# EffortlessMetrics/BitNet-rs

Measured on AMD Instinct MI355X. Metric: decode tokens/sec + I2_S matmul HBM GB/s (% roofline), bitnet-b1.58-2B-4T, higher is better.
Workload: dtype i8 MFMA on producer-quantised activations (QAct: 15-bit fixed point per element, one power-of-two scale per 16), exact integer partial sums, f32 accumulate / f32 elsewhere (f16 embedding table); 1 GPU; bitnet-b1.58-2B-4T I2_S BitNet32-F16 (ternary, one f16 scale per 32 weights), 1xMI355X, batch=1 decode, 128-token prompt; layers=30, prompt_len=128, parallelism=single GPU, launch=hipGraph replay per token, kv_cache=f32 (as the reference, T:1171-1202)

## Files before the change

### bitnet-rs_amd/__init__.py

```python
from __future__ import annotations

import collections
import ctypes as C
import importlib.util
import os
import sys

import numpy as np

HERE = os.path.dirname(os.path.abspath(__file__))
ROOT = os.path.dirname(HERE)
LIB_PATH = os.path.join(HERE, "libbitnet_hip.so")
HEADER_PATH = os.path.join(ROOT, "include", "bitnet_hip.h")

OK = 0
ERR_INVALID_ARGUMENT, ERR_GPU, ERR_UNSUPPORTED, ERR_EXECUTION = -1, -2, -3, -4
KERNEL_AUTO, KERNEL_EXACT, KERNEL_VALU, KERNEL_MFMA, KERNEL_MFMA_TILED = 0, 1, 2, 3, 4
QTYPE_I2S, QTYPE_TL1, QTYPE_TL2 = 0, 1, 2

_u8p = C.POINTER(C.c_uint8)
_i8p = C.POINTER(C.c_int8)
_f32p = C.POINTER(C.c_float)
_sz = C.c_size_t
_vp = C.c_void_p
# ... 18 lines not shown
    spec.loader.exec_module(mod)
    return mod


def build(force: bool = False, verbose: bool = False) -> str:
    return _load_build_module().build(force=force, verbose=verbose)


class DeviceInfo(C.Structure):
    _fields_ = [
        ("device_id", C.c_int32),
        ("name", C.c_char * 128),
        ("gcn_arch", C.c_char * 64),
        ("total_memory", C.c_uint64),
        ("compute_unit_count", C.c_int32),
        ("max_wavefront_size", C.c_int32),
        ("max_shared_memory_per_workgroup", C.c_uint64),
        ("supports_fp16", C.c_int32),
        ("supports_bf16", C.c_int32),
    ]


def _np(a, dtype):
    if isinstance(a, (bytes, bytearray, memoryview)):
        a = np.frombuffer(a, dtype=np.uint8)
    return np.ascontiguousarray(a, dtype=dtype)


def _ptr(t):
    return _vp(t if isinstance(t, int) else t.data_ptr())


def _optr(t):
    return None if t is None else _ptr(t)


class HipLib:

    def __init__(self, path: str = LIB_PATH):
        if not os.path.exists(path):
            raise FileNotFoundError(
                f"{path} not found: build it with __graft_entry__.build() -- there is no fallback path"
            )
        self.path = path
        self.c = C.CDLL(path)
        L = self.c
        L.bitnet_hip_init.argtypes = [C.c_int]
        L.bitnet_hip_cleanup.restype = None
        L.bitnet_hip_get_last_error.restype = C.c_char_p
        L.bitnet_hip_get_device_info.argtypes = [C.c_int, C.POINTER(DeviceInfo)]
        L.bitnet_hip_set_kernel.argtypes = [C.c_int]
        L.bitnet_hip_gemv_qk256.argtypes = [_u8p, _sz, _f32p, _sz, _f32p, _sz, _sz, _sz, _sz]
        L.bitnet_hip_i2s_matmul_f32.argtypes = [_f32p, _sz, _u8p, _sz, _f32p, _sz, _f32p, _sz, _sz, _sz, _sz, _sz]
        L.bitnet_hip_qk256_gemv.argtypes = [_u8p, _sz, _f32p, _sz, _f32p, _sz, _f32p, _sz, _sz, _sz, _sz]
        L.bitnet_hip_matmul_i2s.argtypes = [_i8p, _sz, _u8p, _sz, _f32p, _sz, _sz, _sz, _sz]
        L.bitnet_hip_quantize.argtypes = [_f32p, _sz, _u8p, _sz, _f32p, _sz, C.c_int]
        L.bitnet_hip_dequant_i2s.argtypes = [_u8p, _sz, _sz, _sz, C.c_int, C.c_float, C.c_int, _f32p, _sz]
        L.bitnet_hip_attention.argtypes = [_f32p, _sz, _f32p, _sz, _f32p, _sz, _f32p, _sz, _sz, _sz, _sz, C.c_int, C.c_float]
        L.bitnet_hip_qk256_gemv_batch.argtypes = [C.c_void_p, _sz]
        L.bitnet_hip_weights_upload_qk256.argtypes = [_u8p, _sz, _sz, _sz, _sz, C.POINTER(C.c_uint64)]
        L.bitnet_hip_weights_upload_i2s.argtypes = [_u8p, _sz, _f32p, _sz, _sz, _sz, _sz, C.POINTER(C.c_uint64)]
        L.bitnet_hip_weights_upload_coded.argtypes = [_u8p, _sz, _f32p, _sz, _sz, _sz, _sz, _i8p, C.POINTER(C.c_uint64)]
        L.bitnet_hip_weights_upload_inline_f16.argtypes = [_u8p, _sz, _sz, _sz, _i8p, C.c_int, C.POINTER(C.c_uint64)]
        L.bitnet_hip_weights_free.argtypes = [C.c_uint64]
        L.bitnet_hip_weights_info.argtypes = [C.c_uint64, C.POINTER(_sz), C.POINTER(_sz), C.POINTER(_sz)]
        L.bitnet_hip_gemv_dev.argtypes = [C.c_uint64, _vp, _vp, _vp]
        L.bitnet_hip_matmul_dev.argtypes = [C.c_uint64, _vp, _vp, _sz, _vp]
        L.bitnet_hip_matmul_kernel_dev.argtypes = [C.c_uint64, _vp, _vp, _sz, C.c_int, _vp]
        L.bitnet_hip_add_dev.argtypes = [_vp, _vp, _vp, _sz, _vp]
        L.bitnet_hip_silu_mul_dev.argtypes = [_vp, _vp, _vp, _sz, _sz, _vp]
        L.bitnet_hip_weights_device_bytes.argtypes = [C.c_uint64]
        L.bitnet_hip_weights_device_bytes.restype = _sz
        L.bitnet_hip_weights_trim.argtypes = [C.c_uint64]
        L.bitnet_hip_qact_bytes.argtypes = [_sz]
        L.bitnet_hip_qact_bytes.restype = _sz
        L.bitnet_hip_qact_stats_bytes.argtypes = [_sz]
        L.bitnet_hip_qact_stats_bytes.restype = _sz
        L.bitnet_hip_quantize_act_dev.argtypes = [_vp, _vp, _sz, _vp, _vp, _vp]
        L.bitnet_hip_embed_q_dev.argtypes = [_vp, _vp, _vp, _sz, _sz, _vp, _vp, _vp, _vp, _vp]
        L.bitnet_hip_gemv_q_supported.argtypes = [C.c_uint64]
        L.bitnet_hip_gemv_q_dev.argtypes = [C.c_uint64, _vp, _vp, _vp, C.c_float, _vp, C.c_int, _vp, _vp, _vp, _vp, _vp]
        L.bitnet_hip_attention_decode_q_dev.argtypes = [_vp, _vp, _vp, _vp, _vp, _sz, _sz, _sz, _sz, _vp, _vp, C.c_int, _vp, _vp, _vp]
        L.bitnet_hip_gemv_attn_merge_q_dev.argtypes = [C.c_uint64, _vp, _sz, _sz, _sz, _vp, _vp, _vp, _vp, _vp, _vp, _vp]
        L.bitnet_hip_matmul_workspace_bytes.argtypes = [_sz, _sz, C.c_int]
        L.bitnet_hip_matmul_workspace_bytes.restype = _sz
        L.bitnet_hip_matmul_fused_dev.argtypes = [C.c_uint64, _vp, _vp, _sz, _vp, C.c_float, _vp, C.c_int, C.c_int, _vp, _sz, _vp]
        L.bitnet_hip_matmul_last_tile.argtypes = [C.POINTER(C.c_int)] * 4
        L.bitnet_hip_matmul_last_wave_rows.argtypes = []
        L.bitnet_hip_weights_bind_ln.argtypes = [C.c_uint64, _vp, _vp]
        L.bitnet_hip_weights_concat.argtypes = [C.POINTER(C.c_uint64), _sz, C.c_int, C.POINTER(C.c_uint64)]
        L.bitnet_hip_gemv_fused_dev.argtypes = [C.c_uint64, _vp, _vp, _sz, _vp, C.c_float, _vp, C.c_int, _vp]
        L.bitnet_hip_rmsnorm.argtypes = [_f32p, _sz, _f32p, _sz, _f32p, _sz, _sz, _sz, C.c_float]
        L.bitnet_hip_norm_rows_dev.argtypes = [_vp, _vp, _vp, _sz, _sz, C.c_float, C.c_int, _vp]
        L.bitnet_hip_embed_f16_dev.argtypes = [_vp, _vp, _vp, _sz, _sz, _sz, _vp, _vp]
        L.bitnet_hip_advance_pos_dev.argtypes = [_vp, _vp]
        L.bitnet_hip_attention_decode_dev.argtypes = [_vp, _vp, _vp, _vp, _vp, _sz, _sz, _sz, _sz, _vp, _vp, _vp, _vp]
        L.bitnet_hip_attention_decode_wide_dev.argtypes = [_vp, _vp, _vp, _vp, _vp, _sz, _sz, _sz, _sz, _vp, _vp, _vp, _vp]
        L.bitnet_hip_attention_decode_partial_dev.argtypes = [_vp, _vp, _vp, _vp, _vp, _sz, _sz, _sz, _sz, _vp, _vp, _vp]
        L.bitnet_hip_gemv_attn_merge_dev.argtypes = [C.c_uint64, _vp, _sz, _sz, _sz, _vp, _vp, _vp, _vp]
        L.bitnet_hip_attention_prefill_workspace_bytes.argtypes = [_sz, _sz, _sz]
        L.bitnet_hip_attention_prefill_workspace_bytes.restype = _sz
        L.bitnet_hip_attention_prefill_dev.argtypes = [_vp, _vp, _vp, _vp, _vp, _sz, _sz, _sz, _sz, _sz, _vp, _sz, _vp, _vp]
        L.bitnet_hip_attention_extend_workspace_bytes.argtypes = [_sz, _sz, _sz, _sz]
        L.bitnet_hip_attention_extend_workspace_bytes.restype = _sz
        L.bitnet_hip_attention_extend_dev.argtypes = [_vp, _vp, _vp, _vp, _vp, _sz, _sz, _sz, _sz, _sz, _sz, _vp, _sz, _vp, C.c_int, _vp]
        L.bitnet_hip_attention_prefill_sharded_workspace_bytes.argtypes = [_sz, _sz, _sz, _sz]
        L.bitnet_hip_attention_prefill_sharded_workspace_bytes.restype = _sz
        L.bitnet_hip_attention_prefill_sharded_dev.argtypes = [_vp, _sz, _vp, _sz, _vp, _sz, _sz, _vp, _vp, _vp, _vp, _sz, _sz, _sz, _sz, _vp, _sz, _vp, _vp]
        L.bitnet_hip_attention_scratch_bytes.argtypes = [_sz, _sz]
        L.bitnet_hip_attention_scratch_bytes.restype = _sz
        L.bitnet_hip_logits_f16_dev.argtypes = [_vp, _vp, _vp, C.c_float, _sz, _sz, _vp, _vp, _sz, _vp, _vp, _vp, _vp, _vp]
        L.bitnet_hip_argmax_dev.argtypes = [_vp, _sz, _vp, _sz, _vp, _vp]
        L.bitnet_hip_hbm_read_ceiling.argtypes = [_sz, C.c_int, C.POINTER(C.c_double), C.POINTER(C.c_double), _vp]
        L.bitnet_hip_sampler_create.argtypes = [_sz, C.POINTER(SamplingConfig), C.POINTER(_vp)]
        L.bitnet_hip_sampler_destroy.argtypes = [_vp]
        L.bitnet_hip_sampler_destroy.restype = None
        L.bitnet_hip_sampler_configure.argtypes = [_vp, C.POINTER(SamplingConfig)]
        L.bitnet_hip_sampler_reset.argtypes = [_vp]
        L.bitnet_hip_sampler_draws.argtypes = [_vp, C.POINTER(C.c_uint64)]
        L.bitnet_hip_sample_dev.argtypes = [_vp, _vp, _sz, _vp, _vp, _vp, _vp, _vp]
        L.bitnet_hip_sample_host.argtypes = [_vp, _f32p, _sz, C.POINTER(C.c_uint32), _sz, C.POINTER(C.c_uint32)]
        L.bitnet_hip_score_workspace_bytes.argtypes = [_sz, _sz, _sz]
        L.bitnet_hip_score_workspace_bytes.restype = _sz
        L.bitnet_hip_score_f16_dev.argtypes = [_vp, _vp, _vp, C.c_float, _sz, _sz, _sz, _vp, _vp, _vp, _vp, _sz, _vp, _sz, _vp]

    def last_error(self) -> str:
        e = self.c.bitnet_hip_get_last_error()
        return e.decode() if e else ""

    def _check(self, rc: int) -> None:
        if rc != 0:
            raise BitNetHipError(rc, self.last_error() or f"bitnet_hip rc={rc}")

    def init(self, device: int = -1) -> None:
        self._check(self.c.bitnet_hip_init(device))

    def cleanup(self) -> None:
        self.c.bitnet_hip_cleanup()

    def is_available(self) -> bool:
        return bool(self.c.bitnet_hip_is_available())

    def device_count(self) -> int:
        return int(self.c.bitnet_hip_device_count())

    def device_info(self, device: int = 0) -> DeviceInfo:
        info = DeviceInfo()
        self._check(self.c.bitnet_hip_get_device_info(device, C.byref(info)))
        return info

    def set_kernel(self, kernel: int) -> None:
        self._check(self.c.bitnet_hip_set_kernel(kernel))

    def get_kernel(self) -> int:
        return int(self.c.bitnet_hip_get_kernel())

    def gemv_qk256(self, qs, x, rows, cols, row_stride_bytes, y_len=None) -> np.ndarray:
        q, xa = _np(qs, np.uint8), _np(x, np.float32)
        y = np.zeros(rows if y_len is None else y_len, np.float32)
        self._check(
            self.c.bitnet_hip_gemv_qk256(
                q.ctypes.data_as(_u8p), q.size, xa.ctypes.data_as(_f32p), xa.size, y.ctypes.data_as(_f32p), y.size,
                rows, cols, row_stride_bytes,
            )
        )
        return y
# ... 185 lines not shown
                                                           _vp(stream)))

    def attention_prefill_sharded_workspace_bytes(self, n_heads: int, n_kv: int, n_q: int, n_ctx: int) -> int:
        return int(self.c.bitnet_hip_attention_prefill_sharded_workspace_bytes(n_heads, n_kv, n_q, n_ctx))

    def attention_prefill_sharded_dev(self, q, ld_q, q_block_pos, n_q, kv, ld_kv, n_ctx, rope_sin, rope_cos, kcache, vcache, n_heads, n_kv,
                                      head_dim, max_pos, workspace, workspace_bytes, out, stream: int = 0) -> None:
        self._check(self.c.bitnet_hip_attention_prefill_sharded_dev(_ptr(q), ld_q, _ptr(q_block_pos), n_q, _ptr(kv), ld_kv, n_ctx, _ptr(rope_sin),
                                                                    _ptr(rope_cos), _ptr(kcache), _ptr(vcache), n_heads, n_kv, head_dim, max_pos,
                                                                    _ptr(workspace), workspace_bytes, _ptr(out), _vp(stream)))

    def attention_prefill_gathered_dev(self, q, ld_q, q_block_pos, n_q, kv_gathered, n_ctx, world, kv_is_f16, rope_sin, rope_cos, kcache, vcache,
                                       cache_f16, n_heads, n_kv, head_dim, max_pos, workspace, workspace_bytes, out, stream: int = 0) -> None:
        self.c.bitnet_hip_attention_prefill_gathered_dev.argtypes = [_vp, _sz, _vp, _sz, _vp, _sz, _sz, C.c_int, _vp, _vp, _vp, _vp, C.c_int, _sz, _sz,
                                                                     _sz, _sz, _vp, _sz, _vp, _vp]
        self._check(self.c.bitnet_hip_attention_prefill_gathered_dev(_ptr(q), ld_q, _ptr(q_block_pos), n_q, _ptr(kv_gathered), n_ctx, world,
                                                                     int(kv_is_f16), _ptr(rope_sin), _ptr(rope_cos), _ptr(kcache), _ptr(vcache),
                                                                     int(cache_f16), n_heads, n_kv, head_dim, max_pos, _ptr(workspace), workspace_bytes,
                                                                     _ptr(out), _vp(stream)))

    def weights_bind_ln(self, h: int, ln_gamma, stream: int = 0) -> None:
        self._check(self.c.bitnet_hip_weights_bind_ln(h, _ptr(ln_gamma), _vp(stream)))

    def weights_free(self, h: int) -> None:
        self._check(self.c.bitnet_hip_weights_free(h))

    def weights_info(self, h: int):
        r, c, b = _sz(0), _sz(0), _sz(0)
        self._check(self.c.bitnet_hip_weights_info(h, C.byref(r), C.byref(c), C.byref(b)))
        return r.value, c.value, b.value

    def gemv_dev(self, h: int, x, y, stream: int = 0) -> None:
        self._check(self.c.bitnet_hip_gemv_dev(h, _ptr(x), _ptr(y), _vp(stream)))

    def matmul_dev(self, h: int, x, y, m: int, stream: int = 0) -> None:
        self._check(self.c.bitnet_hip_matmul_dev(h, _ptr(x), _ptr(y), m, _vp(stream)))

    def matmul_kernel_dev(self, h: int, x, y, m: int, kernel: int, stream: int = 0) -> None:
        self._check(self.c.bitnet_hip_matmul_kernel_dev(h, _ptr(x), _ptr(y), m, kernel, _vp(stream)))

    def add_dev(self, a, b, out, n: int, stream: int = 0) -> None:
        self._check(self.c.bitnet_hip_add_dev(_ptr(a), _ptr(b), _ptr(out), n, _vp(stream)))

    def silu_mul_dev(self, gate, up, out, n: int, tile: int = 0, stream: int = 0) -> None:
        self._check(self.c.bitnet_hip_silu_mul_dev(_ptr(gate), _ptr(up), _ptr(out), n, tile, _vp(stream)))

    def weights_device_bytes(self, h: int) -> int:
        return int(self.c.bitnet_hip_weights_device_bytes(h))

    def weights_fp4_image(self, h: int, enable: bool = True, stream: int = 0) -> None:
        self.c.bitnet_hip_weights_fp4_image.argtypes = [C.c_uint64, C.c_int, C.c_void_p]
        self._check(self.c.bitnet_hip_weights_fp4_image(h, 1 if enable else 0, stream))

    def weights_trim(self, h: int) -> None:
        self._check(self.c.bitnet_hip_weights_trim(h))

    def qact_bytes(self, cols: int) -> int:
        return int(self.c.bitnet_hip_qact_bytes(cols))

    def qact_stats_bytes(self, cols: int) -> int:
        return int(self.c.bitnet_hip_qact_stats_bytes(cols))

    def quantize_act_dev(self, x, gamma, cols: int, qact_out, stats_out=None, stream: int = 0) -> None:
        self._check(self.c.bitnet_hip_quantize_act_dev(_ptr(x), _optr(gamma), cols, _ptr(qact_out), _optr(stats_out), _vp(stream)))

    def embed_q_dev(self, table, tokens, x_out, hidden: int, vocab: int, gamma, qact_out, stats_out=None, offset=None, stream: int = 0) -> None:
        self._check(self.c.bitnet_hip_embed_q_dev(_ptr(table), _ptr(tokens), _optr(offset), hidden, vocab, _ptr(x_out), _optr(gamma), _ptr(qact_out),
                                                  _optr(stats_out), _vp(stream)))

    def gemv_q_supported(self, h: int) -> bool:
        return bool(self.c.bitnet_hip_gemv_q_supported(h))

    def gemv_q_dev(self, h: int, qact_in, y=None, stats_in=None, ln_gamma=None, ln_eps: float = 0.0, residual=None, flags: int = 0, qact_out=None,
                   gamma_out=None, stats_out=None, stream: int = 0) -> None:
        self._check(self.c.bitnet_hip_gemv_q_dev(h, _ptr(qact_in), _optr(stats_in), _optr(ln_gamma), ln_eps, _optr(residual), flags, _optr(y),
                                                 _optr(qact_out), _optr(gamma_out), _optr(stats_out), _vp(stream)))

    def attention_decode_q_dev(self, qkv, rope_sin, rope_cos, kcache, vcache, n_heads, n_kv, head_dim, max_pos, pos, scratch, out, qact_out,
                               wide: bool = False, kv_f16: bool = False, stream: int = 0, partial: bool = False) -> None:
        flags = (1 if wide else 0) | (2 if kv_f16 else 0) | (4 if partial else 0)
        self._check(self.c.bitnet_hip_attention_decode_q_dev(_ptr(qkv), _ptr(rope_sin), _ptr(rope_cos), _ptr(kcache), _ptr(vcache), n_heads, n_kv,
                                                             head_dim, max_pos, _ptr(pos), _ptr(scratch), flags, _optr(out), _optr(qact_out), _vp(stream)))

    def gemv_attn_merge_q_dev(self, h: int, scratch, n_heads, n_kv, max_pos, pos, y, qact_out, residual=None, gamma_out=None, stats_out=None,
                              stream: int = 0) -> None:
        self._check(self.c.bitnet_hip_gemv_attn_merge_q_dev(h, _ptr(scratch), n_heads, n_kv, max_pos, _ptr(pos), _ptr(y), _optr(residual),
                                                            _ptr(qact_out), _optr(gamma_out), _optr(stats_out), _vp(stream)))

    def weights_concat(self, parts, interleave16: bool = False) -> int:
        arr = (C.c_uint64 * len(parts))(*parts)
        h = C.c_uint64(0)
        self._check(self.c.bitnet_hip_weights_concat(arr, len(parts), int(interleave16), C.byref(h)))
        return h.value

    def gemv_fused_dev(self, h: int, x, y, m: int = 1, ln_gamma=None, ln_eps: float = 0.0, residual=None, flags: int = 0, stream: int = 0) -> None:
        self._check(
            self.c.bitnet_hip_gemv_fused_dev(h, _ptr(x), _ptr(y), m, _ptr(ln_gamma) if ln_gamma is not None else None, ln_eps,
                                             _ptr(residual) if residual is not None else None, flags, _vp(stream))
        )

    def rmsnorm(self, x, gamma, num_rows: int, hidden: int, eps: float = 1e-6) -> np.ndarray:
        xa, ga = _np(x, np.float32), _np(gamma, np.float32)
        out = np.zeros(num_rows * hidden, np.float32)
        self._check(self.c.bitnet_hip_rmsnorm(xa.ctypes.data_as(_f32p), xa.size, ga.ctypes.data_as(_f32p), ga.size, out.ctypes.data_as(_f32p), out.size, num_rows, hidden, eps))
        return out

    def norm_rows_dev(self, x, gamma, out, rows: int, hidden: int, eps: float, rms: bool, stream: int = 0) -> None:
        self._check(self.c.bitnet_hip_norm_rows_dev(_ptr(x), _ptr(gamma), _ptr(out), rows, hidden, eps, int(rms), _vp(stream)))

    def embed_f16_dev(self, table, tokens, out, n: int, hidden: int, vocab: int, offset=None, stream: int = 0) -> None:
        self._check(self.c.bitnet_hip_embed_f16_dev(_ptr(table), _ptr(tokens), _ptr(offset) if offset is not None else None, n, hidden, vocab, _ptr(out), _vp(stream)))

    def attention_decode_dev(self, qkv, rope_sin, rope_cos, kcache, vcache, n_heads, n_kv, head_dim, max_pos, pos, scratch, out, stream: int = 0) -> None:
        self._check(self.c.bitnet_hip_attention_decode_dev(_ptr(qkv), _ptr(rope_sin), _ptr(rope_cos), _ptr(kcache), _ptr(vcache), n_heads, n_kv, head_dim, max_pos, _ptr(pos), _ptr(scratch), _ptr(out), _vp(stream)))

    def attention_decode_wide_dev(self, qkv, rope_sin, rope_cos, kcache, vcache, n_heads, n_kv, head_dim, max_pos, pos, scratch, out, stream: int = 0) -> None:
        self._check(self.c.bitnet_hip_attention_decode_wide_dev(_ptr(qkv), _ptr(rope_sin), _ptr(rope_cos), _ptr(kcache), _ptr(vcache), n_heads, n_kv, head_dim, max_pos, _ptr(pos), _ptr(scratch), _ptr(out), _vp(stream)))

    def attention_decode_partial_dev(self, qkv, rope_sin, rope_cos, kcache, vcache, n_heads, n_kv, head_dim, max_pos, pos, scratch, stream: int = 0) -> None:
        self._check(self.c.bitnet_hip_attention_decode_partial_dev(_ptr(qkv), _ptr(rope_sin), _ptr(rope_cos), _ptr(kcache), _ptr(vcache), n_heads, n_kv, head_dim, max_pos, _ptr(pos), _ptr(scratch), _vp(stream)))

    def gemv_attn_merge_dev(self, h: int, scratch, n_heads: int, n_kv: int, max_pos: int, pos, y, residual=None, stream: int = 0) -> None:
        self._check(self.c.bitnet_hip_gemv_attn_merge_dev(h, _ptr(scratch), n_heads, n_kv, max_pos, _ptr(pos), _ptr(y), _ptr(residual) if residual is not None else None, _vp(stream)))

    def logits_f16_dev(self, table, x, gamma, eps, hidden, vocab, logits, scratch, n_wg, token=None, pos=None, history=None, n_forced=None, stream: int = 0) -> None:
        opt = lambda t: _ptr(t) if t is not None else None
        self._check(self.c.bitnet_hip_logits_f16_dev(_ptr(table), _ptr(x), opt(gamma), eps, hidden, vocab, _ptr(logits), _ptr(scratch), n_wg, opt(token), opt(pos), opt(history), opt(n_forced), _vp(stream)))

    def score_workspace_bytes(self, n_rows: int, hidden: int, vocab: int) -> int:
        return int(self.c.bitnet_hip_score_workspace_bytes(n_rows, hidden, vocab))

    def score_f16_dev(self, table, x, gamma, eps: float, hidden: int, vocab: int, n_rows: int, targets, nll, argmax=None, logits=None,
                      logits_rows: int = 0, workspace=None, workspace_bytes: int = 0, stream: int = 0) -> None:
        self._check(self.c.bitnet_hip_score_f16_dev(_optr(table), _optr(x), _optr(gamma), eps, hidden, vocab, n_rows, _optr(targets), _optr(nll),
                                                    _optr(argmax), _optr(logits), logits_rows, _optr(workspace), workspace_bytes, _vp(stream)))

    def argmax_dev(self, v, n: int, scratch, n_wg: int, token, stream: int = 0) -> None:
        self._check(self.c.bitnet_hip_argmax_dev(_ptr(v), n, _ptr(scratch), n_wg, _ptr(token), _vp(stream)))

    def sampler(self, vocab: int, temperature: float = 1.0, top_k: int = 0, top_p: float = 1.0, repetition_penalty: float = 1.0,
                seed: int | None = None) -> "Sampler":
        return Sampler(self, vocab, SamplingConfig.make(temperature, top_k, top_p, repetition_penalty, seed))

    def hbm_read_ceiling(self, nbytes: int = 2 << 30, iters: int = 10, stream: int = 0):
        best, mean = C.c_double(0.0), C.c_double(0.0)
        self._check(self.c.bitnet_hip_hbm_read_ceiling(nbytes, iters, C.byref(best), C.byref(mean), _vp(stream)))
        return best.value, mean.value


class SamplingConfig(C.Structure):
    _fields_ = [("temperature", C.c_float), ("top_k", C.c_int32), ("top_p", C.c_float), ("repetition_penalty", C.c_float), ("seed", C.c_uint64)]

    @classmethod
    def make(cls, temperature: float, top_k: int, top_p: float, repetition_penalty: float, seed: int | None = None) -> "SamplingConfig":
        if seed is None:
            seed = int.from_bytes(os.urandom(8), "little")
        return cls(float(temperature), int(top_k), float(top_p), float(repetition_penalty), int(seed) & 0xFFFFFFFFFFFFFFFF)


class Sampler:

    def __init__(self, lib: HipLib, vocab: int, cfg: SamplingConfig):
        self.lib, self.vocab = lib, int(vocab)
        h = _vp()
        lib._check(lib.c.bitnet_hip_sampler_create(vocab, C.byref(cfg), C.byref(h)))
        self.h = h
# ... 112 lines not shown
            self._buf = np.frombuffer(data, np.uint8).copy()
            self.h = L.bitnet_host_gguf_from_memory(self._buf.ctypes.data_as(_u8p), self._buf.size)
        if (path is not None or data is not None) and not self.h:
            raise BitNetHipError(ERR_INVALID_ARGUMENT, self.error() or "GGUF parse failed")

    def error(self) -> str:
        e = self.c.bitnet_host_gguf_error()
        return e.decode(errors="replace") if e else ""

    def close(self) -> None:
        if self.h:
            self.c.bitnet_host_gguf_close(self.h)
            self.h = None

    @property
    def data_start(self) -> int:
        return int(self.c.bitnet_host_gguf_data_start(self.h))

    def tensors(self) -> list:
        out = []
        for i in range(self.c.bitnet_host_gguf_tensor_count(self.h)):
            name = C.create_string_buffer(512)
            shape = (C.c_uint64 * 8)()
            nd, ty, off, size = C.c_uint32(0), C.c_uint32(0), C.c_uint64(0), C.c_uint64(0)
            rc = self.c.bitnet_host_gguf_tensor_info(self.h, i, name, 512, shape, C.byref(nd), C.byref(ty), C.byref(off), C.byref(size))
            if rc != 0:
                raise BitNetHipError(ERR_INVALID_ARGUMENT, self.error())
            out.append({"name": name.value.decode(), "shape": tuple(int(shape[j]) for j in range(nd.value)), "type": ty.value,
                        "offset": off.value, "size": size.value})
        return out

    def config(self) -> dict:
        cfg, f = (C.c_uint64 * 6)(), (C.c_float * 2)()
        if self.c.bitnet_host_gguf_config(self.h, cfg, f) != 0:
            raise BitNetHipError(ERR_INVALID_ARGUMENT, self.error())
        keys = ("vocab", "hidden", "n_layers", "n_heads", "n_kv_heads", "ffn")
        d = {k: int(cfg[i]) for i, k in enumerate(keys)}
        d["rope_theta"] = None if f[0] != f[0] else float(f[0])
        d["eps"] = None if f[1] != f[1] else float(f[1])
        return d

    def detect_i2s_flavor(self, available: int, nelems: int, has_scale_sibling: bool, strict: bool = False) -> str:
        rc = self.c.bitnet_host_gguf_detect_i2s_flavor(available, nelems, int(has_scale_sibling), int(strict))
        if rc < 0:
            raise BitNetHipError(ERR_INVALID_ARGUMENT, self.error())
        return FLAVORS[rc]

    def check_projection(self, idx: int, rows: int, cols: int) -> None:
        if self.c.bitnet_host_gguf_check_projection(self.h, idx, rows, cols) != 0:
            raise BitNetHipError(ERR_INVALID_ARGUMENT, self.error())

    def loader_is_qk256(self, shape, available: int) -> bool:
        sh = (C.c_uint64 * len(shape))(*shape)
        return bool(self.c.bitnet_host_gguf_loader_is_qk256(sh, len(shape), available))


ScoreResult = collections.namedtuple("ScoreResult", "nll argmax logits ms")


class HostDecoder:

    def __init__(self, cfg, path: str = HOST_LIB_PATH):
        if not os.path.exists(path):
            raise FileNotFoundError(f"{path} not found: build it with __graft_entry__.build() -- there is no fallback path")
        load()
        self.c = C.CDLL(path)
        L = self.c
        L.bitnet_host_create.restype = C.c_void_p
        L.bitnet_host_create.argtypes = [C.POINTER(HostConfig)]
        L.bitnet_host_destroy.argtypes = [C.c_void_p]
        L.bitnet_host_error.restype = C.c_char_p
        L.bitnet_host_error.argtypes = [C.c_void_p]
        L.bitnet_host_set_layer_qk256.argtypes = [C.c_void_p, C.c_int, _f32p, _f32p] + [_u8p] * 7
        L.bitnet_host_set_layer_i2s.argtypes = [C.c_void_p, C.c_int, _f32p, _f32p, C.POINTER(_u8p), C.POINTER(_f32p), _sz]
        L.bitnet_host_set_globals.argtypes = [C.c_void_p, C.POINTER(C.c_uint16), _f32p]
        L.bitnet_host_reset.argtypes = [C.c_void_p]
        L.bitnet_host_feed.argtypes = [C.c_void_p, C.POINTER(C.c_int32), C.c_int]
        L.bitnet_host_run.argtypes = [C.c_void_p, C.c_int, C.c_int, C.c_int, C.POINTER(C.c_float)]
        L.bitnet_host_run_reference.argtypes = [C.c_void_p, C.c_int, C.c_int]
        L.bitnet_host_prepare_graphs.argtypes = [C.c_void_p, C.c_int]
        L.bitnet_host_set_act_mode.argtypes = [C.c_void_p, C.c_int]
        L.bitnet_host_act_mode.argtypes = [C.c_void_p]
        L.bitnet_host_position.argtypes = [C.c_void_p]
        L.bitnet_host_last_prefill_path.argtypes = [C.c_void_p]
        L.bitnet_host_saturation_fallbacks.argtypes = [C.c_void_p]
        L.bitnet_host_history.argtypes = [C.c_void_p, C.POINTER(C.c_int32), C.c_int]
        L.bitnet_host_last_logits.argtypes = [C.c_void_p, _f32p]
        L.bitnet_host_last_hidden.argtypes = [C.c_void_p, _f32p]
        L.bitnet_host_probe_gateup.argtypes = [C.c_void_p, C.c_int, C.POINTER(C.c_float), C.POINTER(C.c_double)]
        L.bitnet_host_probe_kernel.argtypes = [C.c_void_p, C.c_int, C.c_int, C.POINTER(C.c_float), C.POINTER(C.c_double)]
        L.bitnet_host_weight_bytes.argtypes = [C.c_void_p]
        L.bitnet_host_weight_bytes.restype = C.c_uint64
        L.bitnet_host_set_sampling.argtypes = [C.c_void_p, C.POINTER(SamplingConfig)]
        L.bitnet_host_sampling_draws.argtypes = [C.c_void_p, C.POINTER(C.c_uint64)]
        L.bitnet_host_score.argtypes = [C.c_void_p, C.c_int, C.c_int, _f32p, C.POINTER(C.c_int32), _f32p, C.c_int, C.POINTER(C.c_float)]
        L.bitnet_host_extend.argtypes = [C.c_void_p, C.c_int, C.c_int, C.c_int, C.POINTER(C.c_float)]
        L.bitnet_host_extend.restype = C.c_int
        L.bitnet_host_rewind.argtypes = [C.c_void_p, C.c_int]
        L.bitnet_host_rewind.restype = C.c_int
        self.cfg = cfg
        self._fed = 0
        hc = HostConfig(**{k: (float(v) if k in ("eps", "rope_theta") else int(v)) for k, v in cfg.asdict().items()})
        self.h = L.bitnet_host_create(C.byref(hc))
        if not self.h:
            raise BitNetHipError(ERR_GPU, "bitnet_host_create failed (allocation)")
        err = self.error()
        if err:
            self.close()
            raise BitNetHipError(ERR_GPU, err)

    def error(self) -> str:
        e = self.c.bitnet_host_error(self.h)
        return e.decode() if e else ""

    def _check(self, rc: int) -> None:
        if rc != 0:
            raise BitNetHipError(rc, self.error() or f"bitnet_host rc={rc}")

    def close(self) -> None:
        if self.h:
            self.c.bitnet_host_destroy(self.h)
            self.h = None

    def load_gguf(self, gguf: "GgufFile") -> None:
        self.c.bitnet_host_load_gguf.argtypes = [C.c_void_p, C.c_void_p]
        self._check(self.c.bitnet_host_load_gguf(self.h, gguf.h))

    def set_layer_qk256(self, layer: int, w: dict) -> None:
        a = [_np(w["attn_norm"], np.float32), _np(w["ffn_norm"], np.float32)] + [_np(w[k], np.uint8) for k in ("q", "k", "v", "o", "gate", "up", "down")]
        self._check(self.c.bitnet_host_set_layer_qk256(self.h, layer, a[0].ctypes.data_as(_f32p), a[1].ctypes.data_as(_f32p), *[x.ctypes.data_as(_u8p) for x in a[2:]]))

    def set_layer_i2s(self, layer: int, w: dict, block: int) -> None:
        names = ("q", "k", "v", "o", "gate", "up", "down")
        ws = [_np(w[k], np.uint8) for k in names]
        ss = [_np(w[k + "_scales"], np.float32) for k in names]
        wp = (_u8p * 7)(*[x.ctypes.data_as(_u8p) for x in ws])
        sp = (_f32p * 7)(*[x.ctypes.data_as(_f32p) for x in ss])
        an, fn = _np(w["attn_norm"], np.float32), _np(w["ffn_norm"], np.float32)
        self._check(self.c.bitnet_host_set_layer_i2s(self.h, layer, an.ctypes.data_as(_f32p), fn.ctypes.data_as(_f32p), wp, sp, block))

    def set_globals(self, g: dict) -> None:
        e, f = _np(g["embed_f16"], np.uint16), _np(g["final_norm"], np.float32)
        self._check(self.c.bitnet_host_set_globals(self.h, e.ctypes.data_as(C.POINTER(C.c_uint16)), f.ctypes.data_as(_f32p)))

    def reset(self) -> None:
        self._check(self.c.bitnet_host_reset(self.h))
        self._fed = 0

    def set_sampling(self, temperature: float | None, top_k: int = 0, top_p: float = 1.0, repetition_penalty: float = 1.0,
                     seed: int | None = None) -> None:
        if temperature is None:
            self._check(self.c.bitnet_host_set_sampling(self.h, None))
            return
        cfg = SamplingConfig.make(temperature, top_k, top_p, repetition_penalty, seed)
        self._check(self.c.bitnet_host_set_sampling(self.h, C.byref(cfg)))

    def sampling_draws(self) -> int:
        d = C.c_uint64(0)
        self._check(self.c.bitnet_host_sampling_draws(self.h, C.byref(d)))
        return int(d.value)

    def feed(self, tokens) -> None:
        t = _np(tokens, np.int32)
        self._check(self.c.bitnet_host_feed(self.h, t.ctypes.data_as(C.POINTER(C.c_int32)), t.size))
        self._fed += int(t.size)

# ... 11 lines not shown

    def act_mode(self) -> int:
        return int(self.c.bitnet_host_act_mode(self.h))

    def trace_step(self, directory: str, with_logits: bool = True) -> None:
        self.c.bitnet_host_trace_step.argtypes = [C.c_void_p, C.c_char_p, C.c_int]
        os.makedirs(directory, exist_ok=True)
        self._check(self.c.bitnet_host_trace_step(self.h, directory.encode(), int(with_logits)))

    def prepare_graphs(self, with_logits: bool = True) -> None:
        self._check(self.c.bitnet_host_prepare_graphs(self.h, int(with_logits)))

    def run_reference(self, n: int, with_logits: bool = True) -> None:
        self._check(self.c.bitnet_host_run_reference(self.h, n, int(with_logits)))

    GATHER_FN = C.CFUNCTYPE(C.c_int, C.c_void_p, C.c_void_p, C.c_void_p, C.c_size_t, C.c_void_p)

    def prefill_sharded(self, n: int, rank: int, world: int, gather=None, with_logits: bool = True, digits: int = 3, wire_f16: bool = True,
                        rccl_comm: int | None = None) -> float:
        L = self.c
        L.bitnet_host_prefill_sharded.argtypes = [C.c_void_p, C.c_int, C.c_int, C.c_int, C.c_void_p, C.c_void_p, C.c_int, C.c_int, C.c_int, C.POINTER(C.c_float)]
        ms = C.c_float(0)
        if rccl_comm is not None:
            fn = C.cast(L.bitnet_host_rccl_allgather, C.c_void_p)
            self._check(L.bitnet_host_prefill_sharded(self.h, n, rank, world, fn, C.c_void_p(rccl_comm), int(with_logits), digits, int(wire_f16), C.byref(ms)))
            return ms.value
        cb = None
        if gather is not None:
            def _cb(ctx, send, recv, nbytes, stream):
                try:
                    return int(gather(send, recv, nbytes, stream) or 0)
                except Exception as e:
                    sys.stderr.write(f"gather callback failed: {e!r}\n")
                    return -1
            cb = self.GATHER_FN(_cb)
        self._check(L.bitnet_host_prefill_sharded(self.h, n, rank, world, C.cast(cb, C.c_void_p) if cb else None, None, int(with_logits), digits,
                                                  int(wire_f16), C.byref(ms)))
        return ms.value

    def set_phase_timing(self, on: bool) -> None:
        self.c.bitnet_host_set_phase_timing.argtypes = [C.c_void_p, C.c_int]
        self._check(self.c.bitnet_host_set_phase_timing(self.h, int(on)))

    def phase_times(self) -> dict:
        out = (C.c_float * 4)()
        self.c.bitnet_host_phase_times.argtypes = [C.c_void_p, C.POINTER(C.c_float)]
        self._check(self.c.bitnet_host_phase_times(self.h, out))
        return {"matmul_us": round(out[0], 1), "attention_us": round(out[1], 1), "gather_wait_us": round(out[2], 1), "gather_us": round(out[3], 1)}

    def prefill(self, n: int, with_logits: bool = True, digits: int = 4) -> float:
        self.c.bitnet_host_prefill.argtypes = [C.c_void_p, C.c_int, C.c_int, C.c_int, C.POINTER(C.c_float)]
        ms = C.c_float(0)
        self._check(self.c.bitnet_host_prefill(self.h, n, int(with_logits), digits, C.byref(ms)))
        return ms.value

    def extend(self, n: int, with_logits: bool = True, digits: int = 2) -> float:
        ms = C.c_float(0)
        self._check(self.c.bitnet_host_extend(self.h, n, int(with_logits), digits, C.byref(ms)))
        return ms.value

    def rewind(self, n: int) -> None:
        self._check(self.c.bitnet_host_rewind(self.h, n))
        self._fed = min(self._fed, int(n))

    def score(self, n: int | None = None, digits: int = 2, logits_rows: int = 0) -> "ScoreResult":
        n = self._fed if n is None else int(n)
        nll = np.zeros(max(n - 1, 0), np.float32)
        am = np.zeros(max(n, 0), np.int32)
        lg = np.zeros((logits_rows, self.cfg.vocab), np.float32) if logits_rows > 0 else None
        ms = C.c_float(0)
        self._check(self.c.bitnet_host_score(self.h, n, digits, nll.ctypes.data_as(_f32p), am.ctypes.data_as(C.POINTER(C.c_int32)),
                                             lg.ctypes.data_as(_f32p) if lg is not None else None, logits_rows, C.byref(ms)))
        return ScoreResult(nll, am, lg, ms.value)

    def last_prefill_path(self) -> int:
        return int(self.c.bitnet_host_last_prefill_path(self.h))

    def saturation_fallbacks(self) -> int:
        return int(self.c.bitnet_host_saturation_fallbacks(self.h))

    def position(self) -> int:
        return int(self.c.bitnet_host_position(self.h))

    def history(self, n: int) -> np.ndarray:
        out = np.zeros(n, np.int32)
        self._check(self.c.bitnet_host_history(self.h, out.ctypes.data_as(C.POINTER(C.c_int32)), n))
        return out

    def last_logits(self) -> np.ndarray:
        out = np.zeros(self.cfg.vocab, np.float32)
        self._check(self.c.bitnet_host_last_logits(self.h, out.ctypes.data_as(_f32p)))
        return out

    def last_hidden(self) -> np.ndarray:
        out = np.zeros(self.cfg.hidden, np.float32)
        self._check(self.c.bitnet_host_last_hidden(self.h, out.ctypes.data_as(_f32p)))
        return out

    def probe_gateup(self, reps: int):
        us, b = C.c_float(0), C.c_double(0)
        self._check(self.c.bitnet_host_probe_gateup(self.h, reps, C.byref(us), C.byref(b)))
        return us.value, b.value

    def probe_kernel(self, kind: int, reps: int):
        us, b = C.c_float(0), C.c_double(0)
        self._check(self.c.bitnet_host_probe_kernel(self.h, kind, reps, C.byref(us), C.byref(b)))
        return us.value, b.value

    def weight_bytes(self) -> int:
        return int(self.c.bitnet_host_weight_bytes(self.h))
```

### bitnet-rs_amd/csrc/abi.hip

```cpp
#include <atomic>
#include <cmath>
#include <cstring>
#include <memory>
#include <mutex>
#include <unordered_map>
#include <vector>

#include "common.hpp"
#include "qact.hpp"

namespace bitnet_hip {

thread_local std::string g_last_error;

namespace {

std::mutex g_mu;
bool g_inited = false;
int g_device = 0;
std::atomic<int> g_kernel{BITNET_HIP_KERNEL_AUTO};
uint64_t g_next_handle = 1;
using WeightsRef = std::shared_ptr<Weights>;
std::unordered_map<uint64_t, WeightsRef> g_weights;

// ... 834 lines not shown
}

int bitnet_hip_add_dev(const float *a_dev, const float *b_dev, float *out_dev, size_t n, void *stream) {
    BH_GUARD_BEGIN
    if (!a_dev || !b_dev || !out_dev) return set_error(BITNET_HIP_ERR_INVALID_ARGUMENT, "Null pointer passed to add_dev");
    if (n == 0) return BITNET_HIP_OK;
    BH_HIP_TRY(launch_add(a_dev, b_dev, out_dev, n, (hipStream_t)stream));
    return BITNET_HIP_OK;
    BH_GUARD_END
}

int bitnet_hip_silu_mul_dev(const float *gate_dev, const float *up_dev, float *out_dev, size_t n, size_t tile, void *stream) {
    BH_GUARD_BEGIN
    if (!gate_dev || !up_dev || !out_dev) return set_error(BITNET_HIP_ERR_INVALID_ARGUMENT, "Null pointer passed to silu_mul_dev");
    if (n == 0) return BITNET_HIP_OK;
    if (tile != 0 && n % tile != 0) return set_error(BITNET_HIP_ERR_INVALID_ARGUMENT, "silu_mul: n %zu is not a multiple of the tile %zu", n, tile);
    BH_HIP_TRY(launch_silu_mul(gate_dev, up_dev, out_dev, n, tile, (hipStream_t)stream));
    return BITNET_HIP_OK;
    BH_GUARD_END
}

int bitnet_hip_embed_f16_dev(const void *table, const int32_t *tokens_dev, const int32_t *offset_dev, size_t n,
                             size_t hidden, size_t vocab, float *out_dev, void *stream) {
    BH_GUARD_BEGIN
    if (!table || !tokens_dev || !out_dev) return set_error(BITNET_HIP_ERR_INVALID_ARGUMENT, "Null pointer passed to embed_f16_dev");
    if (hidden % 8 != 0) return set_error(BITNET_HIP_ERR_INVALID_ARGUMENT, "embed: hidden %zu must be a multiple of 8", hidden);
    BH_HIP_TRY(launch_embed_f16(table, tokens_dev, offset_dev, (int)n, (int)hidden, (int)vocab, out_dev, (hipStream_t)stream));
    return BITNET_HIP_OK;
    BH_GUARD_END
}

int bitnet_hip_attention_decode_dev(const float *qkv, const float *rope_sin, const float *rope_cos, float *kcache,
                                    float *vcache, size_t n_heads, size_t n_kv_heads, size_t head_dim, size_t max_pos,
                                    const int32_t *pos_dev, float *scratch, float *out, void *stream) {
    BH_GUARD_BEGIN
    if (!qkv || !rope_sin || !rope_cos || !kcache || !vcache || !pos_dev || !scratch || !out)
        return set_error(BITNET_HIP_ERR_INVALID_ARGUMENT, "Null pointer passed to attention_decode_dev");
    if (n_kv_heads == 0 || n_heads % n_kv_heads != 0)
        return set_error(BITNET_HIP_ERR_INVALID_ARGUMENT, "num_heads %zu must be divisible by num_key_value_heads %zu", n_heads, n_kv_heads);
    if (head_dim != 128 || n_heads / n_kv_heads > 4)
        return set_error(BITNET_HIP_ERR_UNSUPPORTED, "attention_decode: head_dim %zu / group %zu unsupported (head_dim 128, group <= 4)",
                         head_dim, n_heads / n_kv_heads);
    BH_HIP_TRY(launch_attn_decode(qkv, rope_sin, rope_cos, kcache, vcache, (int)n_heads, (int)n_kv_heads, (int)head_dim,
                                  (int)max_pos, pos_dev, scratch, out, (hipStream_t)stream));
    return BITNET_HIP_OK;
    BH_GUARD_END
}

int bitnet_hip_attention_decode_wide_dev(const float *qkv, const float *rope_sin, const float *rope_cos, float *kcache,
                                         float *vcache, size_t n_heads, size_t n_kv_heads, size_t head_dim, size_t max_pos,
                                         const int32_t *pos_dev, float *scratch, float *out, void *stream) {
    BH_GUARD_BEGIN
    if (!qkv || !rope_sin || !rope_cos || !kcache || !vcache || !pos_dev || !scratch || !out)
        return set_error(BITNET_HIP_ERR_INVALID_ARGUMENT, "Null pointer passed to attention_decode_wide_dev");
    if (n_kv_heads == 0 || n_heads % n_kv_heads != 0)
        return set_error(BITNET_HIP_ERR_INVALID_ARGUMENT, "num_heads %zu must be divisible by num_key_value_heads %zu", n_heads, n_kv_heads);
    if (head_dim != 128 || n_heads / n_kv_heads > 4)
        return set_error(BITNET_HIP_ERR_UNSUPPORTED, "attention_decode: head_dim %zu / group %zu unsupported (head_dim 128, group <= 4)",
                         head_dim, n_heads / n_kv_heads);
    BH_HIP_TRY(launch_attn_decode(qkv, rope_sin, rope_cos, kcache, vcache, (int)n_heads, (int)n_kv_heads, (int)head_dim,
                                  (int)max_pos, pos_dev, scratch, out, (hipStream_t)stream, true, 2));
    return BITNET_HIP_OK;
    BH_GUARD_END
}

int bitnet_hip_attention_decode_partial_dev(const float *qkv, const float *rope_sin, const float *rope_cos, float *kcache,
                                            float *vcache, size_t n_heads, size_t n_kv_heads, size_t head_dim, size_t max_pos,
                                            const int32_t *pos_dev, float *scratch, void *stream) {
    BH_GUARD_BEGIN
    if (!qkv || !rope_sin || !rope_cos || !kcache || !vcache || !pos_dev || !scratch)
        return set_error(BITNET_HIP_ERR_INVALID_ARGUMENT, "Null pointer passed to attention_decode_partial_dev");
    if (n_kv_heads == 0 || n_heads % n_kv_heads != 0)
        return set_error(BITNET_HIP_ERR_INVALID_ARGUMENT, "num_heads %zu must be divisible by num_key_value_heads %zu", n_heads, n_kv_heads);
    if (head_dim != 128 || n_heads / n_kv_heads > 4)
        return set_error(BITNET_HIP_ERR_UNSUPPORTED, "attention_decode: head_dim %zu / group %zu unsupported (head_dim 128, group <= 4)",
                         head_dim, n_heads / n_kv_heads);
    BH_HIP_TRY(launch_attn_decode(qkv, rope_sin, rope_cos, kcache, vcache, (int)n_heads, (int)n_kv_heads, (int)head_dim,
                                  (int)max_pos, pos_dev, scratch, nullptr, (hipStream_t)stream, false));
    return BITNET_HIP_OK;
    BH_GUARD_END
}

size_t bitnet_hip_attention_merge_max_keys(void) { return (size_t)4 * 64; }

static int gemv_attn_merge(bitnet_hip_weights_t h, const float *attn_scratch_dev, size_t n_heads, size_t n_kv_heads, size_t max_pos,
                           const int32_t *pos_dev, float *y_dev, const float *residual_dev, void *qact_out, const float *gamma_out_dev,
                           double *stats_out, void *stream, int chunk_log2 = 6) {
    BH_GUARD_BEGIN
    const WeightsRef w = lookup(h);
    if (!w) return set_error(BITNET_HIP_ERR_INVALID_ARGUMENT, "unknown weights handle %llu", (unsigned long long)h);
    if (!attn_scratch_dev || !pos_dev || !y_dev) return set_error(BITNET_HIP_ERR_INVALID_ARGUMENT, "Null pointer passed to gemv_attn_merge_dev");
    const size_t group = n_kv_heads ? n_heads / n_kv_heads : 0;
    if (n_kv_heads == 0 || n_heads % n_kv_heads != 0 || (group != 1 && group != 2 && group != 4) || w->cols != n_heads * 128)
        return set_error(BITNET_HIP_ERR_UNSUPPORTED, "gemv_attn_merge_dev: needs cols == n_heads * 128 and a query group of 1, 2 or 4 (got %zu heads / %zu)",
                         n_heads, n_kv_heads);
    if (!mfma_supported(*w) || div_ceil(div_ceil(w->cols, 256), (size_t)8) > 2)
        return set_error(BITNET_HIP_ERR_UNSUPPORTED, "gemv_attn_merge_dev: matrix shape %zux%zu not supported", w->rows, w->cols);
    if (qact_out && w->rows % 16 != 0)
        return set_error(BITNET_HIP_ERR_UNSUPPORTED, "gemv_attn_merge_q_dev: rows %zu must be a multiple of 16 for a QAct output", w->rows);
    if (qact_out && gemvq_supported(*w) && w->cols <= 4096) {
        GemvQIo io;
        io.residual = residual_dev;
        io.y = y_dev;
        io.qout = qact_out;
        io.gamma_out = gamma_out_dev;
        io.stats_out = stats_out;
        io.attn_rec = attn_scratch_dev;
        io.attn_pos = pos_dev;
        io.attn_chunk_log2 = chunk_log2;
        io.attn_chunks_max = (int)div_ceil(max_pos, (size_t)1 << chunk_log2);
        io.attn_group_log2 = group == 4 ? 2 : group == 2 ? 1 : 0;
        hipError_t e = launch_gemv_q(*w, io, (hipStream_t)stream);
        if (e != hipSuccess) return set_error(BITNET_HIP_ERR_GPU, "kernel launch failed: %s", hipGetErrorString(e));
        return BITNET_HIP_OK;
    }
    GemvFusion fu;
    fu.residual = residual_dev;
    fu.attn_rec = attn_scratch_dev;
    fu.attn_pos = pos_dev;
    fu.attn_chunk_log2 = chunk_log2;
    fu.attn_chunks_max = (int)div_ceil(max_pos, (size_t)1 << fu.attn_chunk_log2);
    fu.attn_group_log2 = group == 4 ? 2 : group == 2 ? 1 : 0;
    fu.qout = qact_out;
    fu.gamma_out = gamma_out_dev;
    fu.stats_out = stats_out;
    return run_gemv(*w, attn_scratch_dev, y_dev, 1, fu, (hipStream_t)stream, BITNET_HIP_KERNEL_MFMA);
    BH_GUARD_END
}

int bitnet_hip_gemv_attn_merge_dev(bitnet_hip_weights_t h, const float *attn_scratch_dev, size_t n_heads, size_t n_kv_heads,
                                   size_t max_pos, const int32_t *pos_dev, float *y_dev, const float *residual_dev, void *stream) {
    return gemv_attn_merge(h, attn_scratch_dev, n_heads, n_kv_heads, max_pos, pos_dev, y_dev, residual_dev, nullptr, nullptr, nullptr, stream);
}

int bitnet_hip_gemv_attn_merge_q_dev(bitnet_hip_weights_t h, const float *attn_scratch_dev, size_t n_heads, size_t n_kv_heads,
                                     size_t max_pos, const int32_t *pos_dev, float *y_dev, const float *residual_dev, void *qact_out,
                                     const float *gamma_out_dev, double *stats_out, void *stream) {
    if (!qact_out) return set_error(BITNET_HIP_ERR_INVALID_ARGUMENT, "Null pointer passed to gemv_attn_merge_q_dev");
    return gemv_attn_merge(h, attn_scratch_dev, n_heads, n_kv_heads, max_pos, pos_dev, y_dev, residual_dev, qact_out, gamma_out_dev, stats_out, stream);
}


size_t bitnet_hip_qact_bytes(size_t cols) { return qact_bytes(cols); }
size_t bitnet_hip_qact_stats_bytes(size_t cols) { return div_ceil(cols, 16) * 2 * sizeof(double); }

int bitnet_hip_quantize_act_dev(const float *x_dev, const float *gamma_dev, size_t cols, void *qact_out, double *stats_out, void *stream) {
    BH_GUARD_BEGIN
    if (!x_dev || !qact_out) return set_error(BITNET_HIP_ERR_INVALID_ARGUMENT, "Null pointer passed to quantize_act_dev");
    if (cols == 0 || cols % 16 != 0) return set_error(BITNET_HIP_ERR_INVALID_ARGUMENT, "quantize_act: cols %zu must be a positive multiple of 16", cols);
    BH_HIP_TRY(launch_quant_act(x_dev, gamma_dev, cols, qact_out, stats_out, (hipStream_t)stream));
    return BITNET_HIP_OK;
    BH_GUARD_END
}

int bitnet_hip_embed_q_dev(const void *table, const int32_t *tokens_dev, const int32_t *offset_dev, size_t hidden, size_t vocab,
                           float *x_out_dev, const float *gamma_dev, void *qact_out, double *stats_out, void *stream) {
    BH_GUARD_BEGIN
    if (!table || !tokens_dev || !x_out_dev || !qact_out) return set_error(BITNET_HIP_ERR_INVALID_ARGUMENT, "Null pointer passed to embed_q_dev");
    if (hidden == 0 || hidden % 16 != 0) return set_error(BITNET_HIP_ERR_INVALID_ARGUMENT, "embed_q: hidden %zu must be a positive multiple of 16", hidden);
    BH_HIP_TRY(launch_embed_q(table, tokens_dev, offset_dev, (int)hidden, (int)vocab, x_out_dev, gamma_dev, qact_out, stats_out, (hipStream_t)stream));
    return BITNET_HIP_OK;
    BH_GUARD_END
}

int bitnet_hip_gemv_q_supported(bitnet_hip_weights_t h) {
    const WeightsRef w = lookup(h);
    return w && gemvq_supported(*w) ? 1 : 0;
}

int bitnet_hip_gemv_q_dev(bitnet_hip_weights_t h, const void *qact_in, const double *stats_in, const float *ln_gamma_dev, float ln_eps,
                          const float *residual_dev, int flags, float *y_dev, void *qact_out, const float *gamma_out_dev, double *stats_out,
                          void *stream) {
    BH_GUARD_BEGIN
    const WeightsRef w = lookup(h);
    if (!w) return set_error(BITNET_HIP_ERR_INVALID_ARGUMENT, "unknown weights handle %llu", (unsigned long long)h);
    if (!qact_in || (!y_dev && !qact_out)) return set_error(BITNET_HIP_ERR_INVALID_ARGUMENT, "Null pointer passed to gemv_q_dev");
    if (!gemvq_supported(*w))
        return set_error(BITNET_HIP_ERR_UNSUPPORTED, "gemv_q_dev: matrix %zux%zu (block %zu) is not on the QAct path (cols %% 256 == 0, rows %% 16 == 0, no scales or 32-element blocks)",
                         w->rows, w->cols, w->block_size);
    GemvQIo io;
    io.qin = qact_in;
    io.stats_in = stats_in;
    io.ln_gamma = ln_gamma_dev;
    io.ln_eps = ln_eps;
    io.residual = residual_dev;
    io.silu_mul = (flags & BITNET_HIP_FUSE_SILU_MUL) != 0;
    io.y = y_dev;
    io.qout = qact_out;
    io.gamma_out = gamma_out_dev;
    io.stats_out = stats_out;
    if (io.silu_mul && (!w->paired || residual_dev || w->rows % 32 != 0))
        return set_error(BITNET_HIP_ERR_INVALID_ARGUMENT, "FUSE_SILU_MUL needs a handle from weights_concat(..., interleave16=1) and no residual");
    if (ln_gamma_dev && (!stats_in || !w->ln_g || w->ln_gamma_bound != ln_gamma_dev))
        return set_error(BITNET_HIP_ERR_INVALID_ARGUMENT, "gemv_q_dev: LayerNorm needs stats_in and the gamma bound with bitnet_hip_weights_bind_ln");
    if (ln_gamma_dev && w->cols > 4096)
        return set_error(BITNET_HIP_ERR_UNSUPPORTED, "gemv_q_dev: LayerNorm input of %zu columns (<= 4096)", w->cols);
    hipError_t e = launch_gemv_q(*w, io, (hipStream_t)stream);
    if (e != hipSuccess) return set_error(BITNET_HIP_ERR_GPU, "kernel launch failed: %s", hipGetErrorString(e));
    return BITNET_HIP_OK;
    BH_GUARD_END
}

int bitnet_hip_attention_decode_q_dev(const float *qkv, const float *rope_sin, const float *rope_cos, void *kcache, void *vcache,
                                      size_t n_heads, size_t n_kv_heads, size_t head_dim, size_t max_pos, const int32_t *pos_dev,
                                      float *scratch, int flags, float *out, void *qact_out, void *stream) {
    const int wide = (flags & BITNET_HIP_ATTN_WIDE) != 0, kv16 = (flags & BITNET_HIP_ATTN_KV_F16) != 0, partial = (flags & BITNET_HIP_ATTN_PARTIAL) != 0;
    BH_GUARD_BEGIN
    if (!qkv || !rope_sin || !rope_cos || !kcache || !vcache || !pos_dev || !scratch || (!out && !qact_out && !partial))
        return set_error(BITNET_HIP_ERR_INVALID_ARGUMENT, "Null pointer passed to attention_decode_q_dev");
    if (n_kv_heads == 0 || n_heads % n_kv_heads != 0)
        return set_error(BITNET_HIP_ERR_INVALID_ARGUMENT, "num_heads %zu must be divisible by num_key_value_heads %zu", n_heads, n_kv_heads);
    if (head_dim != 128 || n_heads / n_kv_heads > 4)
        return set_error(BITNET_HIP_ERR_UNSUPPORTED, "attention_decode: head_dim %zu / group %zu unsupported (head_dim 128, group <= 4)",
                         head_dim, n_heads / n_kv_heads);
    BH_HIP_TRY(launch_attn_decode(qkv, rope_sin, rope_cos, static_cast<float *>(kcache), static_cast<float *>(vcache), (int)n_heads, (int)n_kv_heads,
                                  (int)head_dim, (int)max_pos, pos_dev, scratch, out, (hipStream_t)stream, !partial, wide ? 2 : 1, qact_out, kv16));
    return BITNET_HIP_OK;
    BH_GUARD_END
}

size_t bitnet_hip_attention_prefill_workspace_bytes(size_t n_heads, size_t n_kv_heads, size_t seq_len) {
    return attn_prefill_workspace_bytes((int)n_heads, (int)n_kv_heads, (int)seq_len, (int)seq_len);
// ... 484 lines not shown
```

### bitnet-rs_amd/csrc/common.hpp

```cpp
#pragma once

#include <hip/hip_runtime.h>

#include <atomic>
#include <cstdarg>
#include <cstdint>
#include <cstdio>
#include <memory>
#include <mutex>
#include <string>

#include "bitnet_hip.h"

namespace bitnet_hip {

extern thread_local std::string g_last_error;

inline int set_error(int code, const char *fmt, ...) __attribute__((format(printf, 2, 3)));
inline int set_error(int code, const char *fmt, ...) {
    char buf[512];
    va_list ap;
    va_start(ap, fmt);
    vsnprintf(buf, sizeof(buf), fmt, ap);
    va_end(ap);
// ... 2 lines not shown
}

#define BH_HIP_TRY(expr)                                                                       \
    do {                                                                                       \
        hipError_t _e = (expr);                                                                \
        if (_e != hipSuccess)                                                                  \
            return ::bitnet_hip::set_error(BITNET_HIP_ERR_GPU, "HIP error %d (%s) at %s:%d: %s", \
                                           (int)_e, hipGetErrorName(_e), __FILE__, __LINE__,   \
                                           #expr);                                             \
    } while (0)

inline size_t div_ceil(size_t a, size_t b) { return (a + b - 1) / b; }

hipError_t raise_dynamic_lds(const void *kernel, int bytes);
template <class... A>
inline hipError_t raise_dynamic_lds(void (*kernel)(A...), int bytes) { return raise_dynamic_lds(reinterpret_cast<const void *>(kernel), bytes); }

constexpr uint32_t pack_lut(int v0, int v1, int v2, int v3) {
    return (uint32_t)(uint8_t)(int8_t)v0 | ((uint32_t)(uint8_t)(int8_t)v1 << 8) |
           ((uint32_t)(uint8_t)(int8_t)v2 << 16) | ((uint32_t)(uint8_t)(int8_t)v3 << 24);
}
constexpr uint32_t LUT_QK256 = pack_lut(-2, -1, 1, 2);
constexpr uint32_t LUT_TERNARY = pack_lut(0, 1, 0, -1);

struct Weights {
    size_t rows = 0;
    size_t cols = 0;
    size_t row_stride_bytes = 0;
    size_t block_size = 0;
    size_t nblk = 0;
    uint32_t lut = 0;
    bool scaled = false;
    uint8_t *codes = nullptr;
    float *scales = nullptr;
    std::shared_ptr<std::mutex> mu = std::make_shared<std::mutex>();
    std::shared_ptr<std::atomic<int>> ref_pins = std::make_shared<std::atomic<int>>(0);
    size_t algorithmic_bytes = 0;
    int device = 0;
    uint8_t *tiles = nullptr;
    uint8_t *tiles4 = nullptr;
    float *scale_tiles = nullptr;
    bool scales_f16 = false;
    bool scales_f16_x2_finite = false;
    uint16_t *scale_tiles_h = nullptr;
    size_t n_row_tiles = 0, n_kblocks = 0;
    bool paired = false;
    float *ln_g = nullptr;
    const float *ln_gamma_bound = nullptr;
};

struct GemvFusion {
    const float *ln_gamma = nullptr;
    float ln_eps = 0.0f;
    const float *residual = nullptr;
    bool silu_mul = false;
    bool x_f16 = false, y_f16 = false;
    bool int8_form = false;
    bool fp6_form = false;
    bool fp6_expand = false;
    const float *attn_rec = nullptr;
    const int *attn_pos = nullptr;
    int attn_chunks_max = 0;
    int attn_chunk_log2 = 6;
    int attn_group_log2 = 0;
    void *qout = nullptr;
    const float *gamma_out = nullptr;
    double *stats_out = nullptr;
};

struct GemvQIo {
    const void *qin = nullptr;
    const double *stats_in = nullptr;
    const float *ln_gamma = nullptr;
    float ln_eps = 0.0f;
    const float *residual = nullptr;
    bool silu_mul = false;
    float *y = nullptr;
    void *qout = nullptr;
    const float *gamma_out = nullptr;
    double *stats_out = nullptr;
    const float *attn_rec = nullptr;
    const int *attn_pos = nullptr;
    int attn_chunks_max = 0, attn_group_log2 = 0, attn_chunk_log2 = 6;
};


hipError_t launch_gemv_exact(const Weights &w, const float *x, float *y, size_t m, hipStream_t stream);
hipError_t launch_gemv_valu(const Weights &w, const float *x, float *y, size_t m, hipStream_t stream);
bool valu_supported(const Weights &w);
hipError_t launch_gemv_mfma(const Weights &w, const float *x, float *y, size_t m, const GemvFusion &fu,
                            hipStream_t stream);
bool mfma_supported(const Weights &w);
int mfma_pick_ksplit(size_t rows, size_t cols, bool paired, int nw);
bool gemvq_supported(const Weights &w);
hipError_t launch_gemv_q(const Weights &w, const GemvQIo &io, hipStream_t stream);
hipError_t launch_quant_act(const float *x, const float *gamma, size_t n, void *qout, double *stats, hipStream_t stream);
hipError_t launch_embed_q(const void *table, const int *tokens, const int *offset_ptr, int hidden, int vocab, float *x_out,
                          const float *gamma, void *qout, double *stats, hipStream_t stream);
hipError_t build_tiles(Weights &w, hipStream_t stream);
hipError_t ensure_reference(Weights &w, hipStream_t stream, bool pin = false, bool scales_only = false);
void trim_reference(Weights &w);
struct ReferencePin {
    Weights &w;
    hipError_t status;
    ReferencePin(Weights &w_, hipStream_t stream, bool scales_only = false) : w(w_), status(ensure_reference(w_, stream, true, scales_only)) {}
    ~ReferencePin() {
        if (status == hipSuccess) w.ref_pins->fetch_sub(1, std::memory_order_acq_rel);
    }
    ReferencePin(const ReferencePin &) = delete;
    ReferencePin &operator=(const ReferencePin &) = delete;
};
size_t weights_device_bytes(const Weights &w);
bool gemm_supported(const Weights &w);
bool gemm_fp6_supported(const Weights &w);
bool gemm_fp4_resident_enabled();
hipError_t ensure_fp4_image(Weights &w, hipStream_t stream);
void drop_fp4_image(Weights &w);
bool gemm_takes_fp6(const Weights &w, const GemvFusion &fu, int ndig);
bool gemm_needs_row_major_scales(const Weights &w);
size_t gemm_workspace_bytes(size_t m, size_t cols, int ndig);
struct GemmF16Io {
    const void *xh = nullptr;
    const float *stats_in = nullptr;
    int n_stats = 0;
    float ln_eps = 0.0f;
    float *y = nullptr;
    const float *residual = nullptr;
    bool silu_mul = false;
    void *yh = nullptr;
    const float *gamma_out = nullptr;
    float *stats_out = nullptr;
    void *qb_out = nullptr;
};
size_t qb32_bytes(size_t m, size_t cols);
hipError_t launch_rows_to_qb32(const float *x, const float *gamma, size_t m, size_t cols, void *qb, float *stats, hipStream_t stream);
bool gemm_qb32_supported(const Weights &w);
hipError_t launch_gemm_qb32(const Weights &w, const GemmF16Io &io, size_t m, hipStream_t stream);
bool gemm_f16_chain_supported(const Weights &w);
unsigned long long f16_saturations(bool reset);
hipError_t launch_gemm_f16_chain(const Weights &w, const GemmF16Io &io, size_t m, hipStream_t stream);
hipError_t launch_rows_to_f16(const float *x, const float *gamma, size_t m, size_t cols, void *xh, float *stats, hipStream_t stream);
hipError_t launch_gemm_mfma(const Weights &w, const float *x, float *y, size_t m, const GemvFusion &fu, int ndig,
                            void *workspace, size_t workspace_bytes, hipStream_t stream);
struct GemmTileChoice {
    int digits = 0, wave_tokens = 0, waves = 0, scale_mode = 0, wave_rows = 64;
    int resident_fp4 = 0;
};
extern thread_local GemmTileChoice g_last_gemm_tile;
extern unsigned long long *g_mfma_stamps;
hipError_t launch_matmul_i2s_u8(const int8_t *a, const uint8_t *b, float *c, size_t m, size_t n,
                                size_t k, hipStream_t stream);
hipError_t launch_quantize_i2s(const float *in, size_t n, uint8_t *out, size_t out_len, float *scales,
                               hipStream_t stream);
bool matmul_i2s_tiled_ok(size_t m, size_t n, size_t k);
hipError_t launch_matmul_i2s_tiled(const int8_t *a, const uint8_t *b, float *c, size_t m, size_t n, size_t k, hipStream_t stream);
hipError_t launch_quantize_i2s_fast(const float *in, size_t n, uint8_t *out, size_t out_len, float *scales, hipStream_t stream);
hipError_t launch_quant_input_i2s(const float *x, int8_t *q, size_t n, hipStream_t stream);
hipError_t launch_unpack_codes_u8(const uint8_t *packed, uint8_t *out, size_t numel, hipStream_t stream);
hipError_t launch_apply_scales(float *out, size_t m, size_t n, const float *scales, size_t n_scales, size_t in_features, size_t block_size,
                               hipStream_t stream);
hipError_t launch_dequant_i2s(const uint8_t *bytes, size_t rows, size_t cols, size_t block, int inv,
                              float k, int transposed, float *out, hipStream_t stream);

hipError_t launch_embed_f16(const void *table, const int *tokens, const int *offset_ptr, int n, int hidden,
                            int vocab, float *out, hipStream_t stream);
hipError_t launch_advance_pos(int *pos_ptr, hipStream_t stream);
// ... 31 lines not shown
```

### bitnet-rs_amd/csrc/kernels_gemvq.hip

```cpp
#include <cstdlib>

#include "common.hpp"
#include "qact.hpp"
#include "wave.hpp"

namespace bitnet_hip {

namespace {

constexpr int kMaxGroupQ = 4;
#ifdef BH_STAMPS
#define BH_QSTAMP(i)                                                                                           \
    do {                                                                                                       \
        if (p.stamps && lane == 0 && (wave == 0 || wave == NW - 1))                                            \
            p.stamps[(size_t)blockIdx.x * 16 + (wave ? 8 : 0) + (i)] = __builtin_amdgcn_s_memrealtime();      \
    } while (0)
#else
#define BH_QSTAMP(i) \
    do {             \
    } while (0)
#endif

struct GemvQArgs {
    const uint8_t *tiles;
    const void *stiles;
    int rows, cols, nblk;
    uint32_t lut;
    int ks_log2;
    const uint8_t *qin;
    const double *stats_in;
    int n_stats;
    const float *ln_g;
    float ln_eps;
    double inv_cols;
    const float *residual;
    float *y;
    int silu_mul;
    uint8_t *qout;
    const float *gamma_out;
    double *stats_out;
    const float *attn_rec;
    const int *attn_pos;
    int attn_chunks_max, attn_group_log2, attn_chunk_log2;
    unsigned long long *stamps;
};

template <int NW, int RING, int SC, int LN, int NCP, int NE = 0>
__global__ __launch_bounds__(NW * 64) void k_gemv_q(GemvQArgs p) {
    constexpr int NT = NW * 64;
    constexpr bool MRG = NE > 0;
    constexpr int ZB = RING * kQRec;
    asm volatile("" ::"s"(p.tiles), "s"(p.stiles), "s"(p.rows), "s"(p.nblk), "s"(p.lut), "s"(p.ks_log2), "s"(p.qin), "s"(p.stats_in), "s"(p.n_stats),
                 "s"(p.ln_g), "s"(p.residual), "s"(p.y), "s"(p.silu_mul), "s"(p.qout), "s"(p.gamma_out), "s"(p.stats_out));
    extern __shared__ __attribute__((aligned(16))) uint8_t lds[];
    const int tid = threadIdx.x, lane = tid & 63;
    const int wave = __builtin_amdgcn_readfirstlane(tid >> 6);
    uint8_t *zq = lds;
    uint8_t *cq = lds + ZB;
    uint8_t *cs = cq + NCP * 16 * NT;
    float *part = reinterpret_cast<float *>(cs + (LN ? NT * 16 : 0));
    BH_QSTAMP(0);
    if (16 * tid < ZB) *reinterpret_cast<v4u *>(zq + 16 * tid) = v4u{0u, 0u, 0u, 0u};

    const int ksplit = 1 << p.ks_log2;
    const int tiles_per_wg = NW >> p.ks_log2;
    const int n_tiles = p.rows >> 4;
    int tile = blockIdx.x * tiles_per_wg + (wave >> p.ks_log2);
    tile = tile < n_tiles ? tile : n_tiles - 1;
    int kpart = wave & (ksplit - 1);
    if (NW == 8 && p.ks_log2 == 3 && wave >= 4) kpart = 11 - wave;
    const int b0 = (kpart * p.nblk) >> p.ks_log2, b1 = ((kpart + 1) * p.nblk) >> p.ks_log2;

    const uint32_t q_last = (uint32_t)kQRec * (uint32_t)p.nblk - 16u;
    v4u qa[NCP];
    float4 mo[MRG ? NE : 1][4];
    float2 mml[MRG ? NE : 1][4];
    if (!MRG) {
#pragma unroll
        for (int i = 0; i < NCP; ++i) qa[i] = *reinterpret_cast<const v4u *>(p.qin + umin32(16u * (uint32_t)(tid + NT * i), q_last));
    } else {
#pragma unroll
        for (int i = 0; i < NE; ++i) {
            int e = 4 * (tid + NT * i);
            e = e < p.cols ? e : p.cols - 4;
            const int h = e >> 7, d = e & 127, kvh = h >> p.attn_group_log2, hg = h & ((1 << p.attn_group_log2) - 1);
            const float *rb = p.attn_rec + (size_t)kvh * p.attn_chunks_max * kAttnRecFloats;
#pragma unroll
            for (int c = 0; c < 4; ++c) {
                const float *rec = rb + (size_t)(c < p.attn_chunks_max ? c : p.attn_chunks_max - 1) * kAttnRecFloats;
                mml[i][c] = *reinterpret_cast<const float2 *>(rec + 2 * hg);
                mo[i][c] = *reinterpret_cast<const float4 *>(rec + 2 * kMaxGroupQ + hg * 128 + d);
            }
        }
    }
    v4u st = {0u, 0u, 0u, 0u};
    if (LN) st = *reinterpret_cast<const v4u *>(p.stats_in + 2 * (size_t)(tid < p.n_stats ? tid : p.n_stats - 1));
    const int e_tl = tid >> 4, e_r = tid & 15;
    int e_row, e_g0 = 0, e_g1 = 0;
    if (!p.silu_mul) {
        e_row = 16 * (blockIdx.x * tiles_per_wg + e_tl) + e_r;
        e_row = e_row < p.rows ? e_row : p.rows - 1;
        e_g0 = e_row;
    } else {
        const int half_rows = p.rows >> 1;
        const int pg = blockIdx.x * (tiles_per_wg >> 1) + e_tl;
        e_row = 16 * pg + e_r;
        e_row = e_row < half_rows ? e_row : half_rows - 1;
        e_g0 = 32 * (e_row >> 4) + e_r;
        e_g1 = e_g0 + 16;
    }
    float e_lg0 = 0.0f, e_lg1 = 0.0f;
    if (LN) {
        e_lg0 = p.ln_g[e_g0];
        e_lg1 = p.ln_g[e_g1];
    }
    const float e_res = (p.residual ? p.residual : reinterpret_cast<const float *>(p.qin))[p.residual ? e_row : 0];
    const float e_gam = (p.gamma_out ? p.gamma_out : reinterpret_cast<const float *>(p.qin))[p.gamma_out ? e_row : 0];
    __builtin_amdgcn_sched_barrier(0);
    const size_t tb0 = (size_t)tile * p.nblk;
    const uint8_t *wbase = p.tiles + (tb0 * 64 + lane) * 16;
    v4u wt[RING];
    uint32_t sh[SC == 2 ? RING : 1];
    float2 sf[SC == 1 ? RING : 1];
#pragma unroll
    for (int j = 0; j < RING; ++j) {
        const int blk = b0 + j < b1 ? b0 + j : b1 - 1;
        wt[j] = load_nt16v(wbase + (size_t)blk * 1024);
        if (SC == 2) sh[j] = __builtin_nontemporal_load(reinterpret_cast<const uint32_t *>(p.stiles) + (tb0 + blk) * 64 + lane);
        if (SC == 1) {
            const float *sp = reinterpret_cast<const float *>(p.stiles) + ((tb0 + blk) * 64 + lane) * 2;
            sf[j] = float2{__builtin_nontemporal_load(sp), __builtin_nontemporal_load(sp + 1)};
        }
    }
    __builtin_amdgcn_sched_barrier(0);
    BH_QSTAMP(1);

    if (!MRG) {
#pragma unroll
        for (int i = 0; i < NCP; ++i) *reinterpret_cast<v4u *>(cq + 16 * (tid + NT * i)) = qa[i];
    } else {
        const int m_chunks = (*p.attn_pos + (1 << p.attn_chunk_log2)) >> p.attn_chunk_log2;
#pragma unroll
        for (int i = 0; i < NE; ++i) {
            const int e = 4 * (tid + NT * i);
            float M = -INFINITY;
#pragma unroll
            for (int c = 0; c < 4; ++c) {
                mml[i][c].x = c < m_chunks ? mml[i][c].x : -INFINITY;
                M = fmaxf(M, mml[i][c].x);
            }
            float L = 0.0f;
            float4 a = {0.0f, 0.0f, 0.0f, 0.0f};
#pragma unroll
            for (int c = 0; c < 4; ++c) {
                const float w = __expf(mml[i][c].x - M);
                L += w * mml[i][c].y;
                a.x += w * mo[i][c].x, a.y += w * mo[i][c].y, a.z += w * mo[i][c].z, a.w += w * mo[i][c].w;
            }
            const float rl = e < p.cols ? 1.0f / L : 0.0f;
            const float v[4] = {a.x * rl, a.y * rl, a.z * rl, a.w * rl};
            uint32_t u = __float_as_uint(fmaxf(fmaxf(fabsf(v[0]), fabsf(v[1])), fmaxf(fabsf(v[2]), fabsf(v[3])))), o;
            o = dpp_u<0xB1>(u), u = o > u ? o : u;
            o = dpp_u<0x4E>(u), u = o > u ? o : u;
            int be = (int)(u >> 23);
            be = be < 32 ? 32 : be;
            be = be > 254 ? 254 : be;
            const float sc = __uint_as_float((uint32_t)(267 - be) << 23), as = __uint_as_float((uint32_t)(be - 13) << 23);
            uint32_t d0 = 0, d1 = 0;
#pragma unroll
            for (int j = 0; j < 4; ++j) {
                const uint32_t t = ((uint32_t)qcvt_rpi(v[j] * sc) + 0x80u) ^ 0x80u;
                d0 |= (t & 0xffu) << (8 * j);
                d1 |= ((t >> 8) & 0xffu) << (8 * j);
            }
            if (e < p.cols) {
                const int grp = e >> 4, rec = grp >> 4, tp = grp & 15;
                uint8_t *qb = cq + kQRec * rec;
                *reinterpret_cast<uint32_t *>(qb + 16 * tp + (e & 15)) = d0;
                *reinterpret_cast<uint32_t *>(qb + 256 + 16 * tp + (e & 15)) = d1;
                if ((e & 15) == 0) reinterpret_cast<float *>(qb + 512)[4 * (tp >> 2) + 2 * (tp & 1) + ((tp & 3) >> 1)] = as;
            }
        }
    }
    if (LN) *reinterpret_cast<v4u *>(cs + 16 * tid) = st;
    asm volatile("s_waitcnt lgkmcnt(0)\n\ts_barrier" ::: "memory");

    const int g = lane >> 4, c = lane & 15;
    const bool mine = (c >> 2) == g;
    const uint8_t *wq = cq + kQRec * b0;
    const uint8_t *live = wq + 256 * ((c >> 1) & 1) + 64 * g;
    const uint8_t *ba0 = (mine && (c & 1) == 0) ? live : zq;
    const uint8_t *ba1 = (mine && (c & 1) == 1) ? live : zq;
    const uint8_t *sa = wq + 512 + 16 * g;
    BH_QSTAMP(2);

    float facc = 0.0f;
#pragma unroll
    for (int j = 0; j < RING; ++j) {
        if (j > 0 && b0 + j >= b1) continue;
        const float4 as = *reinterpret_cast<const float4 *>(sa + kQRec * j);
        const uint32_t wd[4] = {wt[j][0], wt[j][1], wt[j][2], wt[j][3]};
#pragma unroll
        for (int pp = 0; pp < 2; ++pp) {
            v4i acc = {0, 0, 0, 0};
            acc = __builtin_amdgcn_mfma_i32_16x16x64_i8(*reinterpret_cast<const v4i *>(ba0 + kQRec * j + 32 * pp),
                                                        decode16(wd[2 * pp], p.lut), acc, 0, 0, 0);
            acc = __builtin_amdgcn_mfma_i32_16x16x64_i8(*reinterpret_cast<const v4i *>(ba1 + kQRec * j + 32 * pp + 16),
                                                        decode16(wd[2 * pp + 1], p.lut), acc, 0, 0, 0);
            const int i0 = (int)(((uint32_t)acc[2] << 8) + (uint32_t)acc[0]), i1 = (int)(((uint32_t)acc[3] << 8) + (uint32_t)acc[1]);
            float t = (float)i0 * (pp ? as.y : as.x);
            t = fmaf((float)i1, pp ? as.w : as.z, t);
            if (SC == 2)
                facc = pp ? fma_mix_hi(t, sh[j], facc) : fma_mix_lo(t, sh[j], facc);
            else if (SC == 1)
                facc = fmaf(t, pp ? sf[j].y : sf[j].x, facc);
            else
                facc += t;
        }
    }
    {
        float a = facc, b = facc;
        asm volatile("v_nop\n\tv_nop\n\tv_permlane16_swap_b32 %0, %1" : "+v"(a), "+v"(b));
        facc = a + b;
        a = facc, b = facc;
        asm volatile("v_nop\n\tv_nop\n\tv_permlane32_swap_b32 %0, %1" : "+v"(a), "+v"(b));
        facc = a + b;
    }
    if (lane < 16) part[(((wave >> p.ks_log2) << p.ks_log2) + kpart) * 16 + lane] = facc;
    BH_QSTAMP(3);

    const bool storing = wave * 64 < tiles_per_wg * 16;
    double ln_mean = 0.0, ln_rdenom = 1.0;
    if (LN && storing) {
        double s1 = 0.0, s2 = 0.0;
        for (int i = lane; i < p.n_stats; i += 64) {
            const double2 pr = *reinterpret_cast<const double2 *>(cs + 16 * i);
            s1 += pr.x;
            s2 += pr.y;
        }
        s1 = wave64_sum_d_rows_readlane(s1);
        s2 = wave64_sum_d_rows_readlane(s2);
        const double mean_d = s1 * p.inv_cols;
        const double var_d = s2 * p.inv_cols - mean_d * mean_d;
        ln_mean = (double)(float)mean_d;
        const double denom = (double)sqrtf((float)(var_d > 0.0 ? var_d : 0.0) + p.ln_eps);
        double r = __builtin_amdgcn_rcp(denom);
        r = r * (2.0 - denom * r);
        ln_rdenom = r * (2.0 - denom * r);
    }
    __syncthreads();
    BH_QSTAMP(4);
    if (!storing) return;
    const int tl = e_tl, r = e_r;
    if (!p.silu_mul) {
        if (tl >= tiles_per_wg) return;
        const int t_glob = blockIdx.x * tiles_per_wg + tl;
        if (t_glob >= n_tiles) return;
        const int row = 16 * t_glob + r;
        float pv[NW];
#pragma unroll
        for (int kp = 0; kp < NW; ++kp) pv[kp] = part[((tl << p.ks_log2) + (kp < ksplit ? kp : 0)) * 16 + r];
        float v = 0.0f;
#pragma unroll
// ... 48 lines not shown
    int tok = tokens[offset_ptr ? *offset_ptr : 0];
    tok = tok < 0 ? 0 : tok >= vocab ? vocab - 1 : tok;
    const float v = (float)table[(size_t)tok * hidden + i];
    x_out[i] = v;
    qact_emit(qout, stats, i >> 4, i & 15, v, gamma ? v * gamma[i] : v);
}

}

bool gemvq_supported(const Weights &w) {
    if (!mfma_supported(w)) return false;
    if (w.cols % 256 != 0 || w.rows % 16 != 0) return false;
    if (w.scaled && w.block_size != 32) return false;
    return true;
}

hipError_t launch_quant_act(const float *x, const float *gamma, size_t n, void *qout, double *stats, hipStream_t stream) {
    if (n == 0 || n % 16 != 0) return hipErrorInvalidValue;
    hipLaunchKernelGGL(k_quant_act, dim3((unsigned)div_ceil(n, 256)), dim3(256), 0, stream, x, gamma, (int)n, static_cast<uint8_t *>(qout), stats);
    return hipGetLastError();
}

hipError_t launch_embed_q(const void *table, const int *tokens, const int *offset_ptr, int hidden, int vocab, float *x_out,
                          const float *gamma, void *qout, double *stats, hipStream_t stream) {
    if (hidden <= 0 || hidden % 16 != 0) return hipErrorInvalidValue;
    hipLaunchKernelGGL(k_embed_q, dim3((unsigned)div_ceil((size_t)hidden, 256)), dim3(256), 0, stream, static_cast<const _Float16 *>(table), tokens,
                       offset_ptr, hidden, vocab, x_out, gamma, static_cast<uint8_t *>(qout), stats);
    return hipGetLastError();
}

hipError_t launch_gemv_q(const Weights &w, const GemvQIo &io, hipStream_t stream) {
    if (!w.tiles || !gemvq_supported(w) || (!io.qin && !io.attn_rec)) return hipErrorInvalidValue;
    const bool sc_any = w.scaled;
    const int sc = !sc_any ? 0 : w.scales_f16 ? 2 : 1;
    if (sc == 2 && !w.scale_tiles_h) return hipErrorInvalidValue;
    if (sc == 1 && !w.scale_tiles) return hipErrorInvalidValue;
    GemvQArgs a;
    a.tiles = w.tiles;
    a.stiles = sc == 2 ? (const void *)w.scale_tiles_h : sc == 1 ? (const void *)w.scale_tiles : nullptr;
    a.rows = (int)w.rows;
    a.cols = (int)w.cols;
    a.nblk = (int)(w.cols / 256);
    a.lut = w.lut;
    const int nw = 8;
    const int ksplit = mfma_pick_ksplit(w.rows, w.cols, io.silu_mul, 8);
    a.ks_log2 = ksplit == 8 ? 3 : ksplit == 4 ? 2 : ksplit == 2 ? 1 : 0;
    a.qin = static_cast<const uint8_t *>(io.qin);
    const bool ln = io.ln_gamma != nullptr;
    if (ln && !(w.ln_g && w.ln_gamma_bound == io.ln_gamma && io.stats_in)) return hipErrorInvalidValue;
    a.stats_in = io.stats_in;
    a.n_stats = (int)(w.cols / 16);
    a.ln_g = w.ln_g;
    a.ln_eps = io.ln_eps;
    a.inv_cols = 1.0 / (double)w.cols;
    a.residual = io.residual;
    a.y = io.y;
    a.silu_mul = io.silu_mul ? 1 : 0;
    a.qout = static_cast<uint8_t *>(io.qout);
    a.gamma_out = io.gamma_out;
    a.stats_out = io.stats_out;
    a.attn_rec = io.attn_rec;
    a.attn_pos = io.attn_pos;
    a.attn_chunks_max = io.attn_chunks_max;
    a.attn_group_log2 = io.attn_group_log2;
    a.attn_chunk_log2 = io.attn_chunk_log2;
    a.stamps = g_mfma_stamps;
    if (io.silu_mul && (!w.paired || io.residual)) return hipErrorInvalidValue;
    const int tiles_per_wg = nw / ksplit;
    const unsigned grid = (unsigned)div_ceil(w.rows / 16, (size_t)tiles_per_wg);
    const int ring = (int)div_ceil((size_t)a.nblk, (size_t)ksplit);
    const size_t qbytes = (size_t)kQRec * a.nblk;
    const int ncp = (int)div_ceil(qbytes, (size_t)16 * nw * 64);
    if (ring > 5 || ncp > 3 || (ln && a.n_stats > nw * 64)) return hipErrorInvalidValue;
    void (*kfn)(GemvQArgs) = nullptr;
#define BH_QPICK2(RINGv, NCPv)                                                                                                        \
    if (!kfn && ring <= RINGv && ncp == NCPv)                                                                                         \
        kfn = ln ? (sc == 2 ? k_gemv_q<8, RINGv, 2, 1, NCPv> : sc == 1 ? k_gemv_q<8, RINGv, 1, 1, NCPv> : k_gemv_q<8, RINGv, 0, 1, NCPv>)  \
                 : (sc == 2 ? k_gemv_q<8, RINGv, 2, 0, NCPv> : sc == 1 ? k_gemv_q<8, RINGv, 1, 0, NCPv> : k_gemv_q<8, RINGv, 0, 0, NCPv>);
#define BH_QPICK(RINGv) BH_QPICK2(RINGv, 1) BH_QPICK2(RINGv, 2) BH_QPICK2(RINGv, 3)
    BH_QPICK(2) BH_QPICK(3) BH_QPICK(4) BH_QPICK(5)
#undef BH_QPICK
#undef BH_QPICK2
    if (io.attn_rec) {
        const int ne = (int)div_ceil(w.cols / 4, (size_t)512);
        if (ln || nw != 8 || ring > 2 || ncp != 1 || w.cols % 128 != 0 || ne > 2 || !io.attn_pos || io.attn_chunks_max < 1) return hipErrorInvalidValue;
#define BH_QMRG(NEv)                                                                                                                   \
    if (ne <= NEv && !kfn) kfn = sc == 2 ? k_gemv_q<8, 2, 2, 0, 1, NEv> : sc == 1 ? k_gemv_q<8, 2, 1, 0, 1, NEv> : k_gemv_q<8, 2, 0, 0, 1, NEv>;
        kfn = nullptr;
        BH_QMRG(1) BH_QMRG(2)
#undef BH_QMRG
    }
    if (!kfn) return hipErrorInvalidValue;
    const int ring_t = ring <= 2 ? 2 : ring;
    const size_t lds = (size_t)ring_t * kQRec + (size_t)ncp * 16 * nw * 64 + (ln ? (size_t)nw * 64 * 16 : 0) + (size_t)nw * 16 * sizeof(float);
    hipLaunchKernelGGL(kfn, dim3(grid), dim3(nw * 64), lds, stream, a);
    return hipGetLastError();
}

}
```

### bitnet-rs_amd/host/decoder.cpp

```cpp
#include "decoder.hpp"

#include "blake3.hpp"

#include <hip/hip_runtime_api.h>

#include <dlfcn.h>

#include <cmath>
#include <cstdlib>
#include <cstdio>
#include <cstring>
#include <algorithm>
#include <vector>

namespace bitnet_host {

namespace {
struct Event {
    hipEvent_t e = nullptr;
    ~Event() {
        if (e) hipEventDestroy(e);
    }
};
}

#define HCHK(expr)                                                                     \
    do {                                                                               \
        hipError_t _e = (expr);                                                        \
        if (_e != hipSuccess) {                                                        \
            char _b[256];                                                              \
            snprintf(_b, sizeof(_b), "HIP error %s at %s:%d (%s)", hipGetErrorName(_e), __FILE__, __LINE__, #expr); \
            err_ = _b;                                                                 \
            return BITNET_HIP_ERR_GPU;                                                 \
        }                                                                              \
    } while (0)
#define BCHK(expr)                       \
    do {                                 \
        int _rc = (expr);                \
        if (_rc != 0) return fail(#expr); \
    } while (0)

int Decoder::fail_arg(const char *what) {
    err_ = what;
    return BITNET_HIP_ERR_INVALID_ARGUMENT;
}

int Decoder::fail(const char *what) {
    const char *e = bitnet_hip_get_last_error();
    err_ = std::string(what) + ": " + (e ? e : "error");
    return BITNET_HIP_ERR_EXECUTION;
}

template <class T>
static hipError_t dalloc(T **p, size_t n) {
    return hipMalloc(reinterpret_cast<void **>(p), n * sizeof(T) ? n * sizeof(T) : 1);
}

static std::string config_problem(const Config &c) {
    char b[160];
    if (c.hidden <= 0 || c.n_layers <= 0 || c.n_heads <= 0 || c.n_kv_heads <= 0 || c.head_dim <= 0 || c.ffn <= 0 || c.vocab <= 0 || c.max_pos <= 1) {
        snprintf(b, sizeof(b), "config: every dimension must be positive (hidden %d, layers %d, heads %d/%d, head_dim %d, ffn %d, vocab %d, max_pos %d)",
                 c.hidden, c.n_layers, c.n_heads, c.n_kv_heads, c.head_dim, c.ffn, c.vocab, c.max_pos);
        return b;
    }
    if (c.n_heads % c.n_kv_heads != 0) return "config: num_heads must be divisible by num_key_value_heads";
    if (c.head_dim != 128) return "config: head_dim must be 128 (attention kernels)";
    if (c.n_heads / c.n_kv_heads > 4) return "config: at most 4 query heads per KV head (attention kernels)";
    if (c.hidden % 512 != 0 || c.hidden > 8192) return "config: hidden must be a multiple of 512, <= 8192 (logits kernel)";
    if (c.n_layers > 4096 || c.max_pos > (1 << 20)) return "config: n_layers / max_pos out of range";
    return "";
}

Decoder::Decoder(const Config &cfg) : c_(cfg), layers_(cfg.n_layers > 0 && cfg.n_layers <= 4096 ? (size_t)cfg.n_layers : 0) {
    dead_ = true;
    err_ = config_problem(cfg);
    if (!err_.empty()) {
        layers_.clear();
        return;
    }
    if (const char *e = getenv("BITNET_HOST_LOGITS_WGS")) logits_wgs_ = atoi(e) > 0 ? atoi(e) : logits_wgs_;
    if (const char *e = getenv("BITNET_TRACE_DIR")) trace_dir_ = e;
    if (const char *e = getenv("BITNET_HOST_KV16")) kv_f16_ = atoi(e) != 0;
    if (const char *e = getenv("BITNET_HOST_ACT")) act_mode_ = atoi(e) != 0 ? 1 : 0;
    if (const char *e = getenv("BITNET_HOST_PREFILL_CHAIN")) prefill_chain_ = atoi(e) != 0 ? 1 : 0;
    if (bitnet_hip_init(-1) != 0) {
        const char *e = bitnet_hip_get_last_error();
        err_ = e ? e : "bitnet_hip_init failed";
        return;
    }
    hipStream_t s;
    if (hipStreamCreateWithFlags(&s, hipStreamNonBlocking) != hipSuccess) {
        err_ = "hipStreamCreate failed";
        return;
    }
    stream_ = s;
    const size_t H = c_.hidden, D = c_.head_dim, half = D / 2;
    {
        const int group = c_.n_kv_heads > 0 ? c_.n_heads / c_.n_kv_heads : 0;
        merge_ok_ = c_.head_dim == 128 && (group == 1 || group == 2 || group == 4) && c_.n_heads % c_.n_kv_heads == 0 &&
                    (size_t)c_.n_heads * 128 <= 4096;
    }
    bool ok = true;
    ok &= dalloc(&x_, H) == hipSuccess && dalloc(&x2_, H) == hipSuccess;
    ok &= dalloc(&qkv_, (size_t)(c_.n_heads + 2 * c_.n_kv_heads) * D) == hipSuccess;
    ok &= dalloc(&att_, (size_t)c_.n_heads * D) == hipSuccess;
    ok &= dalloc(&h_, (size_t)c_.ffn) == hipSuccess;
    {
        const size_t qh = bitnet_hip_qact_bytes(H), qq = bitnet_hip_qact_bytes((size_t)c_.n_heads * D), qf = bitnet_hip_qact_bytes((size_t)c_.ffn);
        const size_t sb = bitnet_hip_qact_stats_bytes(H);
        ok = ok && hipMalloc(&qa_x_, qh) == hipSuccess && hipMalloc(&qa_x2_, qh) == hipSuccess && hipMalloc(&qa_att_, qq) == hipSuccess &&
             hipMalloc(&qa_h_, qf) == hipSuccess && hipMalloc((void **)&st_x_, sb) == hipSuccess && hipMalloc((void **)&st_x2_, sb) == hipSuccess;
        ok = ok && hipMemset(qa_x_, 0, qh) == hipSuccess && hipMemset(qa_x2_, 0, qh) == hipSuccess && hipMemset(qa_att_, 0, qq) == hipSuccess &&
             hipMemset(qa_h_, 0, qf) == hipSuccess && hipMemset(st_x_, 0, sb) == hipSuccess && hipMemset(st_x2_, 0, sb) == hipSuccess;
    }
    ok &= dalloc(&ref_n_, H > (size_t)c_.ffn ? H : (size_t)c_.ffn) == hipSuccess && dalloc(&ref_gu_, 2 * (size_t)c_.ffn) == hipSuccess &&
          dalloc(&ref_t_, H) == hipSuccess;
    ok &= dalloc(&logits_, (size_t)c_.vocab) == hipSuccess;
    ok &= hipMalloc(&scratch_, 8 * (size_t)logits_wgs_) == hipSuccess;
    {
        const size_t sb = bitnet_hip_attention_scratch_bytes((size_t)c_.n_kv_heads, (size_t)c_.max_pos);
        ok = ok && hipMalloc((void **)&attn_scratch_, sb) == hipSuccess && hipMemset(attn_scratch_, 0, sb) == hipSuccess;
    }
    ok &= dalloc(&pos_, 1) == hipSuccess && dalloc(&n_forced_, 1) == hipSuccess && dalloc(&token_, 1) == hipSuccess;
    ok &= dalloc(&history_, (size_t)c_.max_pos + 2) == hipSuccess;
    ok &= dalloc(&rope_sin_, (size_t)c_.max_pos * half) == hipSuccess;
    ok &= dalloc(&rope_cos_, (size_t)c_.max_pos * half) == hipSuccess;
    for (auto &L : layers_) {
        const size_t n = (size_t)c_.n_kv_heads * (((size_t)c_.max_pos + 63) / 64 * 64) * D;
        ok &= dalloc(&L.kcache, n) == hipSuccess && dalloc(&L.vcache, n) == hipSuccess;
        ok = ok && hipMemset(L.kcache, 0, n * sizeof(float)) == hipSuccess && hipMemset(L.vcache, 0, n * sizeof(float)) == hipSuccess;
        ok &= dalloc(&L.attn_norm, H) == hipSuccess && dalloc(&L.ffn_norm, H) == hipSuccess;
    }
    ok &= dalloc(&final_norm_, H) == hipSuccess;
    if (!ok) {
        err_ = "device allocation failed";
        return;
    }
    std::vector<float> sn((size_t)c_.max_pos * half), cs((size_t)c_.max_pos * half), inv(half);
    for (size_t i = 0; i < half; ++i) inv[i] = 1.0f / powf(c_.rope_theta, (2.0f * (float)i) / (float)D);
    for (int p = 0; p < c_.max_pos; ++p)
        for (size_t i = 0; i < half; ++i) {
            const float angle = (float)p * inv[i];
            sn[(size_t)p * half + i] = sinf(angle);
            cs[(size_t)p * half + i] = cosf(angle);
        }
    if (hipMemcpy(rope_sin_, sn.data(), sn.size() * 4, hipMemcpyHostToDevice) != hipSuccess ||
        hipMemcpy(rope_cos_, cs.data(), cs.size() * 4, hipMemcpyHostToDevice) != hipSuccess)
        err_ = "rope table upload failed";
    if (!err_.empty()) return;
    dead_ = false;
    reset();
}

Decoder::~Decoder() {
    drop_graphs();
    if (sampler_) bitnet_hip_sampler_destroy(sampler_);
    for (auto &L : layers_) {
        for (bitnet_hip_weights_t h : {L.qkv, L.o, L.gateup, L.down})
            if (h) bitnet_hip_weights_free(h);
        for (float *p : {L.attn_norm, L.ffn_norm, L.kcache, L.vcache})
            if (p) hipFree(p);
    }
    for (void *p : {(void *)embed_, (void *)final_norm_, (void *)rope_sin_, (void *)rope_cos_, (void *)x_, (void *)x2_,
                    (void *)qkv_, (void *)att_, (void *)h_, (void *)ref_n_, (void *)ref_gu_, (void *)ref_t_, qa_x_, qa_x2_, qa_att_, qa_h_, (void *)st_x_, (void *)st_x2_, (void *)logits_, scratch_, (void *)attn_scratch_, (void *)pos_, (void *)n_forced_,
                    (void *)history_, (void *)token_})
        if (p) hipFree(p);
    for (void *p : {(void *)pf_x_, (void *)pf_qkv_, (void *)pf_att_, (void *)pf_h_, pf_gemm_ws_, pf_attn_ws_, sp_kv_send_, sp_kv_all_,
                    (void *)sp_block_pos_, (void *)sp_tokens_, pf_xh_, pf_atth_, pf_hh_, (void *)pf_stats_, pf_qb_, (void *)sc_tgt_, (void *)sc_am_,
                    (void *)sc_nll_, (void *)sc_logits_, sc_ws_})
        if (p) hipFree(p);
    for (void *e : sp_tev_)
        if (e) hipEventDestroy((hipEvent_t)e);
    if (sp_ev_pack_) hipEventDestroy((hipEvent_t)sp_ev_pack_);
    if (sp_ev_gather_) hipEventDestroy((hipEvent_t)sp_ev_gather_);
    if (comm_stream_) hipStreamDestroy((hipStream_t)comm_stream_);
    if (stream_) hipStreamDestroy((hipStream_t)stream_);
}

void Decoder::release_layer(Layer &L) {
    for (bitnet_hip_weights_t *h : {&L.qkv, &L.o, &L.gateup, &L.down}) {
        if (!*h) continue;
        size_t ab = 0;
        if (bitnet_hip_weights_info(*h, nullptr, nullptr, &ab) == 0) weight_bytes_ -= ab < weight_bytes_ ? ab : weight_bytes_;
// ... 140 lines not shown

int Decoder::set_layer_specs(int layer, const float *attn_norm, const float *ffn_norm, const ProjSpec p[7]) {
    if (layer < 0 || (size_t)layer >= layers_.size()) return fail_arg("layer index out of range");
    Layer &L = layers_[(size_t)layer];
    const size_t H = c_.hidden, QD = (size_t)c_.n_heads * c_.head_dim, KD = (size_t)c_.n_kv_heads * c_.head_dim, F = c_.ffn;
    const size_t n[7] = {QD, KD, KD, H, F, F, H}, k[7] = {H, H, H, QD, H, H, F};
    if (p[0].qk256 != p[1].qk256 || p[0].qk256 != p[2].qk256 || p[4].qk256 != p[5].qk256) {
        err_ = "q|k|v (and gate|up) must share one I2_S flavour to be fused";
        return BITNET_HIP_ERR_INVALID_ARGUMENT;
    }
    release_layer(L);
    HCHK(hipMemcpy(L.attn_norm, attn_norm, H * 4, hipMemcpyHostToDevice));
    HCHK(hipMemcpy(L.ffn_norm, ffn_norm, H * 4, hipMemcpyHostToDevice));
    bitnet_hip_weights_t h[7] = {0};
    for (int i = 0; i < 7; ++i) {
        int rc;
        if (p[i].qk256) {
            const size_t stride = (k[i] + 255) / 256 * 64;
            rc = bitnet_hip_weights_upload_qk256(p[i].bytes, p[i].len, n[i], k[i], stride, &h[i]);
        } else {
            rc = bitnet_hip_weights_upload_coded(p[i].bytes, p[i].len, p[i].scales, p[i].n_scales, n[i], k[i], p[i].block, p[i].code_map, &h[i]);
        }
        if (rc != 0) {
            rc = fail("weights upload");
            for (int j = 0; j < i; ++j) bitnet_hip_weights_free(h[j]);
            return rc;
        }
    }
    return adopt_projections(L, h);
}

int Decoder::set_globals(const uint16_t *embed_f16, const float *final_norm) {
    const size_t n = (size_t)c_.vocab * c_.hidden * 2;
    if (!embed_) HCHK(hipMalloc(&embed_, n));
    HCHK(hipMemcpy(embed_, embed_f16, n, hipMemcpyHostToDevice));
    HCHK(hipMemcpy(final_norm_, final_norm, (size_t)c_.hidden * 4, hipMemcpyHostToDevice));
    return 0;
}

int Decoder::reset() {
    host_forced_ = 0;
    if (sampler_) BCHK(bitnet_hip_sampler_reset(sampler_));
    HCHK(hipMemset(pos_, 0, 4));
    HCHK(hipMemset(n_forced_, 0, 4));
    HCHK(hipMemset(history_, 0, ((size_t)c_.max_pos + 2) * 4));
    return 0;
}

int Decoder::feed(const int32_t *tokens, int n) {
    const int p = position();
    if (p < 0) return BITNET_HIP_ERR_GPU;
    const int base = p > host_forced_ ? p : host_forced_;
    if (n < 0 || (n > 0 && !tokens)) {
        err_ = "feed: null tokens";
        return BITNET_HIP_ERR_INVALID_ARGUMENT;
    }
    for (int i = 0; i < n; ++i)
        if (tokens[i] < 0 || tokens[i] >= c_.vocab) {
            char b[96];
            snprintf(b, sizeof(b), "token id %d out of range [0, %d)", tokens[i], c_.vocab);
            err_ = b;
            return BITNET_HIP_ERR_INVALID_ARGUMENT;
        }
    if (base + n > c_.max_pos) {
        err_ = "KV cache overflow";
        return BITNET_HIP_ERR_INVALID_ARGUMENT;
    }
    HCHK(hipMemcpy(history_ + base, tokens, (size_t)n * 4, hipMemcpyHostToDevice));
    host_forced_ = base + n;
    HCHK(hipMemcpy(n_forced_, &host_forced_, 4, hipMemcpyHostToDevice));
    return 0;
}

int Decoder::position() {
    int p = -1;
    if (hipMemcpy(&p, pos_, 4, hipMemcpyDeviceToHost) != hipSuccess) {
        err_ = "position readback failed";
        return -1;
    }
    return p;
}

int Decoder::attn_launch(Layer &L, int form, float *out, void *qout) {
    const int flags = (form >= 2 ? BITNET_HIP_ATTN_WIDE : 0) | ((form & 1) ? BITNET_HIP_ATTN_PARTIAL : 0) | (kv_f16_ ? BITNET_HIP_ATTN_KV_F16 : 0);
    BCHK(bitnet_hip_attention_decode_q_dev(qkv_, rope_sin_, rope_cos_, L.kcache, L.vcache, (size_t)c_.n_heads, (size_t)c_.n_kv_heads, (size_t)c_.head_dim,
                                           (size_t)c_.max_pos, pos_, attn_scratch_, flags, out, qout, stream_));
    return 0;
}

int Decoder::set_kv_f16(bool on) {
    if (position() != 0 || host_forced_ != 0) {
        err_ = "set_kv_f16: only on a fresh sequence (reset() first): a cache is f16 or f32 for its whole life";
        return BITNET_HIP_ERR_INVALID_ARGUMENT;
    }
    if (on != kv_f16_) {
        drop_graphs();
        for (auto &L : layers_) {
            const size_t n = (size_t)c_.n_kv_heads * (((size_t)c_.max_pos + 63) / 64 * 64) * c_.head_dim;
            HCHK(hipMemset(L.kcache, 0, n * sizeof(float)));
            HCHK(hipMemset(L.vcache, 0, n * sizeof(float)));
        }
    }
    kv_f16_ = on;
    return 0;
}

struct Decoder::Tracer {
    std::string dir;
    int seq = 0;
    void *stream = nullptr;
    std::string err;
    bool dump(const std::string &name, const char *stage, int layer, const float *dev, size_t n) {
        std::vector<float> h(n);
        if (hipStreamSynchronize((hipStream_t)stream) != hipSuccess || hipMemcpy(h.data(), dev, n * 4, hipMemcpyDeviceToHost) != hipSuccess) {
            err = "trace: read-back failed";
            return false;
        }
        double ss = 0.0;
        for (float v : h) ss += (double)v * (double)v;
        const double rms = std::sqrt(ss / (double)n);
        std::string file = name;
        for (char &c : file)
            if (c == '/' || c == '\\') c = '_';
        FILE *f = fopen((dir + "/" + file + ".trace").c_str(), "w");
        if (!f) {
            err = "trace: cannot write into " + dir;
            return false;
        }
        fprintf(f, "{\n  \"name\": \"%s\",\n  \"shape\": [\n    1,\n    %zu\n  ],\n  \"dtype\": \"F32\",\n  \"blake3\": \"%s\",\n  \"rms\": %.17g,\n"
                   "  \"num_elements\": %zu,\n  \"seq\": %d,\n  \"layer\": %d,\n  \"stage\": \"%s\"\n}",
                name.c_str(), n, Blake3::hex(h.data(), n * 4).c_str(), rms, n, seq, layer, stage);
        fclose(f);
        return true;
    }
};
#define TRACE(name, stage, layer, ptr, n)                                   \
    do {                                                                    \
        if (tr && !tr->dump(name, stage, layer, ptr, n)) {                  \
            err_ = tr->err;                                                 \
            return BITNET_HIP_ERR_EXECUTION;                                \
        }                                                                   \
    } while (0)

int Decoder::step_launches(bool with_logits, int form, Tracer *tr) {
    void *s = stream_;
    const size_t H = c_.hidden;
    const size_t tQD = (size_t)c_.n_heads * c_.head_dim, tKD = (size_t)c_.n_kv_heads * c_.head_dim;
    const std::string tp = tr ? "t" + std::to_string(tr->seq) + "/" : "";
    if (tr && (form & 1)) form -= 1;
    if (qact_path()) {
        const size_t NH = (size_t)c_.n_heads, NK = (size_t)c_.n_kv_heads, MP = (size_t)c_.max_pos;
        BCHK(bitnet_hip_embed_q_dev(embed_, history_, pos_, H, (size_t)c_.vocab, x_, layers_[0].attn_norm, qa_x_, st_x_, s));
        TRACE(tp + "embeddings", "embeddings", -1, x_, H);
        for (size_t l = 0; l < layers_.size(); ++l) {
            Layer &L = layers_[l];
            const std::string bp = tp + "blk" + std::to_string(l) + "/";
            BCHK(bitnet_hip_gemv_q_dev(L.qkv, qa_x_, st_x_, L.attn_norm, c_.eps, nullptr, 0, qkv_, nullptr, nullptr, nullptr, s));
            TRACE(bp + "q_proj", "q_proj", (int)l, qkv_, tQD);
            TRACE(bp + "k_proj", "k_proj", (int)l, qkv_ + tQD, tKD);
            TRACE(bp + "v_proj", "v_proj", (int)l, qkv_ + tQD + tKD, tKD);
            if (form == 1) {
                if (int rc = attn_launch(L, 1, nullptr, nullptr)) return rc;
                BCHK(bitnet_hip_gemv_attn_merge_q_dev(L.o, attn_scratch_, NH, NK, MP, pos_, x2_, x_, qa_x2_, L.ffn_norm, st_x2_, s));
            } else {
                if (int rc = attn_launch(L, form, tr ? att_ : nullptr, qa_att_)) return rc;
                TRACE(bp + "attn_out", "attn_out", (int)l, att_, tQD);
                BCHK(bitnet_hip_gemv_q_dev(L.o, qa_att_, nullptr, nullptr, 0.f, x_, 0, x2_, qa_x2_, L.ffn_norm, st_x2_, s));
            }
            TRACE(bp + "attn_residual", "attn_residual", (int)l, x2_, H);
            BCHK(bitnet_hip_gemv_q_dev(L.gateup, qa_x2_, st_x2_, L.ffn_norm, c_.eps, nullptr, BITNET_HIP_FUSE_SILU_MUL, tr ? h_ : nullptr, qa_h_, nullptr, nullptr, s));
            TRACE(bp + "ffn_hidden", "ffn_hidden", (int)l, h_, (size_t)c_.ffn);
            const bool more = l + 1 < layers_.size();
            BCHK(bitnet_hip_gemv_q_dev(L.down, qa_h_, nullptr, nullptr, 0.f, x2_, 0, x_, more ? qa_x_ : nullptr, more ? layers_[l + 1].attn_norm : nullptr,
                                       more ? st_x_ : nullptr, s));
            TRACE(bp + "ffn_out", "ffn_out", (int)l, x_, H);
        }
        if (tr) TRACE("t" + std::to_string(tr->seq) + "_all_layers_out", "all_layers_out", -1, x_, H);
        if (with_logits) {
            if (int rc = pick_token(s)) return rc;
            TRACE(tp + "logits", "logits", -1, logits_, (size_t)c_.vocab);
        } else {
            BCHK(bitnet_hip_advance_pos_dev(pos_, s));
        }
        return 0;
    }
    BCHK(bitnet_hip_embed_f16_dev(embed_, history_, pos_, 1, H, (size_t)c_.vocab, x_, s));
    TRACE(tp + "embeddings", "embeddings", -1, x_, H);
    for (size_t l = 0; l < layers_.size(); ++l) {
        Layer &L = layers_[l];
        const std::string bp = tp + "blk" + std::to_string(l) + "/";
        BCHK(bitnet_hip_gemv_fused_dev(L.qkv, x_, qkv_, 1, L.attn_norm, c_.eps, nullptr, 0, s));
        TRACE(bp + "q_proj", "q_proj", (int)l, qkv_, tQD);
        TRACE(bp + "k_proj", "k_proj", (int)l, qkv_ + tQD, tKD);
        TRACE(bp + "v_proj", "v_proj", (int)l, qkv_ + tQD + tKD, tKD);
        if (form == 2) {
            if (int rc = attn_launch(L, 2, att_, nullptr)) return rc;
            TRACE(bp + "attn_out", "attn_out", (int)l, att_, tQD);
            BCHK(bitnet_hip_gemv_fused_dev(L.o, att_, x2_, 1, nullptr, 0.f, x_, 0, s));
        } else if (form == 1) {
            if (int rc = attn_launch(L, 1, nullptr, nullptr)) return rc;
            BCHK(bitnet_hip_gemv_attn_merge_dev(L.o, attn_scratch_, (size_t)c_.n_heads, (size_t)c_.n_kv_heads, (size_t)c_.max_pos, pos_, x2_, x_, s));
        } else {
            if (int rc = attn_launch(L, 0, att_, nullptr)) return rc;
            TRACE(bp + "attn_out", "attn_out", (int)l, att_, tQD);
            BCHK(bitnet_hip_gemv_fused_dev(L.o, att_, x2_, 1, nullptr, 0.f, x_, 0, s));
        }
        TRACE(bp + "attn_residual", "attn_residual", (int)l, x2_, H);
        BCHK(bitnet_hip_gemv_fused_dev(L.gateup, x2_, h_, 1, L.ffn_norm, c_.eps, nullptr, BITNET_HIP_FUSE_SILU_MUL, s));
        TRACE(bp + "ffn_hidden", "ffn_hidden", (int)l, h_, (size_t)c_.ffn);
        BCHK(bitnet_hip_gemv_fused_dev(L.down, h_, x_, 1, nullptr, 0.f, x2_, 0, s));
        TRACE(bp + "ffn_out", "ffn_out", (int)l, x_, H);
    }
    if (tr) TRACE("t" + std::to_string(tr->seq) + "_all_layers_out", "all_layers_out", -1, x_, H);
    if (with_logits) {
        if (int rc = pick_token(s)) return rc;
        TRACE(tp + "logits", "logits", -1, logits_, (size_t)c_.vocab);
    } else {
        BCHK(bitnet_hip_advance_pos_dev(pos_, s));
    }
    return 0;
}

int Decoder::trace_step(const char *dir, bool with_logits) {
    if (!embed_) {
        err_ = "model globals not set";
        return BITNET_HIP_ERR_INVALID_ARGUMENT;
    }
    if (!dir || !*dir) {
        err_ = "trace_step: no directory";
        return BITNET_HIP_ERR_INVALID_ARGUMENT;
    }
    const int p = position();
    if (p < 0) return BITNET_HIP_ERR_GPU;
    if (p + 1 > c_.max_pos - 1) {
        err_ = "KV cache overflow";
        return BITNET_HIP_ERR_INVALID_ARGUMENT;
    }
    if (!with_logits && p + 1 > host_forced_) {
        err_ = "trace_step(with_logits = false) past the fed tokens";
        return BITNET_HIP_ERR_INVALID_ARGUMENT;
    }
    Tracer tr;
    tr.dir = dir;
    tr.seq = p;
    tr.stream = stream_;
    const int rc = step_launches(with_logits, form_at(p), &tr);
    if (rc) return rc;
    HCHK(hipStreamSynchronize((hipStream_t)stream_));
    return 0;
}

int Decoder::step_launches_reference(bool with_logits) {
    void *s = stream_;
    const size_t H = c_.hidden, F = c_.ffn;
    const int K = BITNET_HIP_KERNEL_EXACT;
    BCHK(bitnet_hip_embed_f16_dev(embed_, history_, pos_, 1, H, (size_t)c_.vocab, x_, s));
    for (auto &L : layers_) {
        BCHK(bitnet_hip_norm_rows_dev(x_, L.attn_norm, ref_n_, 1, H, c_.eps, 0, s));
        BCHK(bitnet_hip_matmul_kernel_dev(L.qkv, ref_n_, qkv_, 1, K, s));
        if (int rc = attn_launch(L, 0, att_, nullptr)) return rc;
        BCHK(bitnet_hip_matmul_kernel_dev(L.o, att_, ref_t_, 1, K, s));
        BCHK(bitnet_hip_add_dev(x_, ref_t_, x2_, H, s));
        BCHK(bitnet_hip_norm_rows_dev(x2_, L.ffn_norm, ref_n_, 1, H, c_.eps, 0, s));
        BCHK(bitnet_hip_matmul_kernel_dev(L.gateup, ref_n_, ref_gu_, 1, K, s));
        BCHK(bitnet_hip_silu_mul_dev(ref_gu_, ref_gu_ + 16, h_, F, 16, s));
        BCHK(bitnet_hip_matmul_kernel_dev(L.down, h_, ref_t_, 1, K, s));
        BCHK(bitnet_hip_add_dev(x2_, ref_t_, x_, H, s));
    }
    if (with_logits) {
        if (int rc = pick_token(s)) return rc;
    } else {
        BCHK(bitnet_hip_advance_pos_dev(pos_, s));
    }
    return 0;
}

int Decoder::run_reference(int n, bool with_logits) {
    if (!embed_) {
        err_ = "model globals not set";
        return BITNET_HIP_ERR_INVALID_ARGUMENT;
    }
    if (c_.ffn % 16 != 0) {
        err_ = "run_reference: ffn must be a multiple of 16";
        return BITNET_HIP_ERR_UNSUPPORTED;
    }
    const int p = position();
    if (p < 0) return BITNET_HIP_ERR_GPU;
    if (p + n > c_.max_pos - 1) {
        err_ = "KV cache overflow";
        return BITNET_HIP_ERR_INVALID_ARGUMENT;
    }
    for (int i = 0; i < n; ++i) {
        const int rc = step_launches_reference(with_logits);
        if (rc) return rc;
    }
    HCHK(hipStreamSynchronize((hipStream_t)stream_));
    for (auto &L : layers_)
        for (bitnet_hip_weights_t h : {L.qkv, L.o, L.gateup, L.down})
            if (h) bitnet_hip_weights_trim(h);
    return 0;
}

int Decoder::form_at(int pos) const {
    static const bool merge_env = !(getenv("BITNET_HOST_ATTN_MERGE") && atoi(getenv("BITNET_HOST_ATTN_MERGE")) == 0);
    static const bool wide_env = !(getenv("BITNET_HOST_ATTN_WIDE") && atoi(getenv("BITNET_HOST_ATTN_WIDE")) == 0);
    const int keys = pos + 1;
    if (merge_env && merge_ok_ && keys <= (int)bitnet_hip_attention_merge_max_keys()) return 1;
    if (wide_env && c_.n_kv_heads * ((keys + 63) / 64) > 256) return 2;
    return 0;
}

int Decoder::prepare_graphs(bool with_logits) {
    if (!embed_) {
        err_ = "model globals not set";
        return BITNET_HIP_ERR_INVALID_ARGUMENT;
    }
    unsigned forms = 0;
    for (int pos = 0; pos + 1 < c_.max_pos; ++pos) forms |= 1u << form_at(pos);
    for (int f = 0; f < kGraphs / 2; ++f)
        if (forms & (1u << f))
            if (int rc = ensure_graph(with_logits, f)) return rc;
    return 0;
}

int Decoder::ensure_graph(bool with_logits, int form) {
    const int gi = 2 * form + (with_logits ? 1 : 0);
    if (graph_exec_[gi]) return 0;
    hipStream_t s = (hipStream_t)stream_;
    hipGraph_t g = nullptr;
    HCHK(hipStreamBeginCapture(s, hipStreamCaptureModeGlobal));
    const int rc = step_launches(with_logits, form);
    const hipError_t e = hipStreamEndCapture(s, &g);
    if (rc != 0) {
        if (g) hipGraphDestroy(g);
        return rc;
    }
    HCHK(e);
    hipGraphExec_t ex = nullptr;
    HCHK(hipGraphInstantiate(&ex, g, nullptr, nullptr, 0));
    graph_[gi] = g;
    graph_exec_[gi] = ex;
    return 0;
}

int Decoder::run(int n, bool with_logits, bool use_graph, float *elapsed_ms) {
    if (!embed_) {
        err_ = "model globals not set";
        return BITNET_HIP_ERR_INVALID_ARGUMENT;
    }
    const int p = position();
    if (p < 0) return BITNET_HIP_ERR_GPU;
    if (p + n > c_.max_pos - 1) {
        err_ = "KV cache overflow";
        return BITNET_HIP_ERR_INVALID_ARGUMENT;
    }
    if (!with_logits && p + n > host_forced_) {
        err_ = "run(with_logits = false) past the fed tokens: nothing would choose the next token";
        return BITNET_HIP_ERR_INVALID_ARGUMENT;
    }
    if (!trace_dir_.empty()) {
        for (int i = 0; i < n; ++i) {
            const int rc = trace_step(trace_dir_.c_str(), with_logits);
            if (rc) return rc;
        }
        if (elapsed_ms) *elapsed_ms = 0.f;
        return 0;
    }
    hipStream_t s = (hipStream_t)stream_;
    if (use_graph) {
        for (int i = 0; i < n; ++i) {
            int rc = ensure_graph(with_logits, form_at(p + i));
            if (rc) return rc;
        }
    }
    Event ev0, ev1;
    HCHK(hipEventCreate(&ev0.e));
    HCHK(hipEventCreate(&ev1.e));
    hipEvent_t e0 = ev0.e, e1 = ev1.e;
    HCHK(hipEventRecord(e0, s));
    for (int i = 0; i < n; ++i) {
        if (use_graph) {
            HCHK(hipGraphLaunch((hipGraphExec_t)graph_exec_[2 * form_at(p + i) + (with_logits ? 1 : 0)], s));
        } else {
            int rc = step_launches(with_logits, form_at(p + i));
            if (rc) return rc;
        }
    }
    HCHK(hipEventRecord(e1, s));
    HCHK(hipStreamSynchronize(s));
    float ms = 0.f;
// ... 803 lines not shown
    bitnet_host::LayerWeightsI2s w;
    w.attn_norm = attn_norm;
    w.ffn_norm = ffn_norm;
    for (int i = 0; i < 7; ++i) {
        w.w[i] = w7[i];
        w.scales[i] = scales7[i];
    }
    w.block_size = block_size;
    LIVE(BITNET_HIP_ERR_INVALID_ARGUMENT);
    return D->set_layer_i2s(layer, w);
}
int bitnet_host_set_globals(void *d, const uint16_t *embed_f16, const float *final_norm) {
    LIVE(BITNET_HIP_ERR_INVALID_ARGUMENT);
    return D->set_globals(embed_f16, final_norm);
}
int bitnet_host_reset(void *d) { LIVE(BITNET_HIP_ERR_INVALID_ARGUMENT); return D->reset(); }
int bitnet_host_set_sampling(void *d, const bitnet_hip_sampling_config *cfg) { LIVE(BITNET_HIP_ERR_INVALID_ARGUMENT); return D->set_sampling(cfg); }
int bitnet_host_sampling_draws(void *d, uint64_t *out) { LIVE(BITNET_HIP_ERR_INVALID_ARGUMENT); return D->sampling_draws(out); }
int bitnet_host_feed(void *d, const int32_t *tokens, int n) { LIVE(BITNET_HIP_ERR_INVALID_ARGUMENT); return D->feed(tokens, n); }
int bitnet_host_set_kv_f16(void *d, int on) { LIVE(BITNET_HIP_ERR_INVALID_ARGUMENT); return D->set_kv_f16(on != 0); }
int bitnet_host_set_act_mode(void *d, int mode) { LIVE(BITNET_HIP_ERR_INVALID_ARGUMENT); return D->set_act_mode(mode); }
int bitnet_host_act_mode(void *d) { LIVE(0); return D->qact_path() ? 1 : 0; }
int bitnet_host_prepare_graphs(void *d, int with_logits) { LIVE(BITNET_HIP_ERR_INVALID_ARGUMENT); return D->prepare_graphs(with_logits != 0); }
int bitnet_host_run_reference(void *d, int n, int with_logits) { LIVE(BITNET_HIP_ERR_INVALID_ARGUMENT); return D->run_reference(n, with_logits != 0); }
int bitnet_host_run(void *d, int n, int with_logits, int use_graph, float *elapsed_ms) {
    LIVE(BITNET_HIP_ERR_INVALID_ARGUMENT);
    return D->run(n, with_logits != 0, use_graph != 0, elapsed_ms);
}
int bitnet_host_prefill(void *d, int n, int with_logits, int digits, float *elapsed_ms) {
    LIVE(BITNET_HIP_ERR_INVALID_ARGUMENT);
    return D->prefill(n, with_logits != 0, digits, elapsed_ms);
}
int bitnet_host_extend(void *d, int n, int with_logits, int digits, float *elapsed_ms) {
    LIVE(BITNET_HIP_ERR_INVALID_ARGUMENT);
    return D->extend(n, with_logits != 0, digits, elapsed_ms);
}
int bitnet_host_rewind(void *d, int n) {
    LIVE(BITNET_HIP_ERR_INVALID_ARGUMENT);
    return D->rewind(n);
}
int bitnet_host_prefill_sharded(void *d, int n, int rank, int world, bitnet_host_allgather_fn gather, void *gather_ctx, int with_logits,
                                int digits, int wire_f16, float *elapsed_ms) {
    LIVE(BITNET_HIP_ERR_INVALID_ARGUMENT);
    return D->prefill_sharded(n, rank, world, gather, gather_ctx, with_logits != 0, digits, wire_f16 != 0, elapsed_ms);
}
int bitnet_host_rccl_allgather(void *nccl_comm, const void *send_dev, void *recv_dev, size_t bytes_per_rank, void *stream) {
    using fn_t = int (*)(const void *, void *, size_t, int, void *, void *);
    static fn_t fn = [] {
        void *h = dlopen("librccl.so", RTLD_NOW | RTLD_GLOBAL);
        if (!h) h = dlopen("librccl.so.1", RTLD_NOW | RTLD_GLOBAL);
        return h ? reinterpret_cast<fn_t>(dlsym(h, "ncclAllGather")) : nullptr;
    }();
    if (!fn || !nccl_comm) return -1;
    return fn(send_dev, recv_dev, bytes_per_rank,  1, nccl_comm, stream);
}
int bitnet_host_set_phase_timing(void *d, int on) {
    LIVE(BITNET_HIP_ERR_INVALID_ARGUMENT);
    D->set_phase_timing(on != 0);
    return 0;
}
int bitnet_host_phase_times(void *d, float out[4]) {
    LIVE(BITNET_HIP_ERR_INVALID_ARGUMENT);
    if (!out) return BITNET_HIP_ERR_INVALID_ARGUMENT;
    D->phase_times(out);
    return 0;
}
int bitnet_host_finish_prefill(void *d, int n, const float *last_row, int with_logits) {
    LIVE(BITNET_HIP_ERR_INVALID_ARGUMENT);
    return D->finish_prefill(n, last_row, with_logits != 0);
}
int bitnet_host_score(void *d, int n, int digits, float *nll_out, int32_t *argmax_out, float *logits_out, int logits_rows, float *elapsed_ms) {
    LIVE(BITNET_HIP_ERR_INVALID_ARGUMENT);
    return D->score(n, digits, nll_out, argmax_out, logits_out, logits_rows, elapsed_ms);
}
void bitnet_host_layer_objects(void *d, int layer, uint64_t *handles4, void **ptrs4) {
    for (int i = 0; i < 4; ++i) handles4[i] = 0, ptrs4[i] = nullptr;
    if (Decoder *D = live(d)) D->layer_objects(layer, handles4, ptrs4);
}
void bitnet_host_global_objects(void *d, void **ptrs7) {
    for (int i = 0; i < 7; ++i) ptrs7[i] = nullptr;
    if (Decoder *D = live(d)) D->global_objects(ptrs7);
}
int bitnet_host_position(void *d) { LIVE(-1); return D->position(); }
int bitnet_host_last_prefill_path(void *d) { LIVE(-1); return D->last_prefill_path(); }
int bitnet_host_saturation_fallbacks(void *d) { LIVE(-1); return D->saturation_fallbacks(); }
int bitnet_host_history(void *d, int32_t *out, int n) { LIVE(BITNET_HIP_ERR_INVALID_ARGUMENT); return D->history(out, n); }
int bitnet_host_last_logits(void *d, float *out) { LIVE(BITNET_HIP_ERR_INVALID_ARGUMENT); return D->last_logits(out); }
int bitnet_host_last_hidden(void *d, float *out) { LIVE(BITNET_HIP_ERR_INVALID_ARGUMENT); return D->last_hidden(out); }
int bitnet_host_blake3_hex(const void *data, size_t len, char *out65) {
    if (!out65 || (!data && len)) return -1;
    const std::string h = bitnet_host::Blake3::hex(data, len);
    memcpy(out65, h.c_str(), 65);
    return 0;
}
int bitnet_host_trace_step(void *d, const char *dir, int with_logits) { LIVE(BITNET_HIP_ERR_INVALID_ARGUMENT); return D->trace_step(dir, with_logits != 0); }
int bitnet_host_probe_gateup(void *d, int reps, float *us_per_launch, double *bytes_per_launch) {
    LIVE(BITNET_HIP_ERR_INVALID_ARGUMENT);
    return D->probe_gateup(reps, us_per_launch, bytes_per_launch);
}
int bitnet_host_probe_kernel(void *d, int kind, int reps, float *us_per_launch, double *bytes_per_launch) {
    LIVE(BITNET_HIP_ERR_INVALID_ARGUMENT);
    return D->probe_kernel(kind, reps, us_per_launch, bytes_per_launch);
}
uint64_t bitnet_host_weight_bytes(void *d) { LIVE(0); return D->weight_bytes(); }
}
```

### bitnet-rs_amd/host/decoder.hpp

```cpp
#pragma once

#include <cstddef>
#include <cstdint>
#include <string>
#include <vector>

#include "bitnet_hip.h"

extern "C" {
typedef int (*bitnet_host_allgather_fn)(void *ctx, const void *send_dev, void *recv_dev, size_t bytes_per_rank, void *stream);
}

namespace bitnet_host {

struct Config {
    int hidden = 2560, n_layers = 30, n_heads = 20, n_kv_heads = 5, head_dim = 128;
    int ffn = 6912, vocab = 128256, max_pos = 4096;
    float eps = 1e-5f;
    float rope_theta = 10000.f;
};

struct LayerWeightsQk256 {
    const float *attn_norm, *ffn_norm;
    const uint8_t *q, *k, *v, *o, *gate, *up, *down;
// ... 4 lines not shown
    const float *scales[7];
    size_t block_size;
};

struct ProjSpec {
    bool qk256 = true;
    const uint8_t *bytes = nullptr;
    size_t len = 0;
    const float *scales = nullptr;
    size_t n_scales = 0, block = 32;
    int8_t code_map[4] = {-2, -1, 0, 1};
};

class Decoder {
  public:
    explicit Decoder(const Config &cfg);
    ~Decoder();
    Decoder(const Decoder &) = delete;
    Decoder &operator=(const Decoder &) = delete;

    const Config &config() const { return c_; }
    const std::string &error() const { return err_; }
    bool dead() const { return dead_; }
    void set_error(const std::string &e) { err_ = e; }

    int set_layer_qk256(int layer, const LayerWeightsQk256 &w);
    int set_layer_i2s(int layer, const LayerWeightsI2s &w);
    int set_layer_specs(int layer, const float *attn_norm, const float *ffn_norm, const ProjSpec p[7]);
    int set_globals(const uint16_t *embed_f16, const float *final_norm);

    int reset();
    int set_sampling(const bitnet_hip_sampling_config *cfg);
    int sampling_draws(uint64_t *out);
    int feed(const int32_t *tokens, int n);
    int run(int n, bool with_logits, bool use_graph, float *elapsed_ms);
    int run_reference(int n, bool with_logits);
    int set_act_mode(int mode);
    int set_kv_f16(bool on);
    bool kv_f16() const { return kv_f16_; }
    bool qact_path() const;
    int prefill(int n, bool with_logits, int digits, float *elapsed_ms);
    int extend(int n, bool with_logits, int digits, float *elapsed_ms);
    int rewind(int n);
    int prefill_sharded(int n, int rank, int world, bitnet_host_allgather_fn gather, void *gather_ctx, bool with_logits, int digits,
                        bool wire_f16, float *elapsed_ms);
    int finish_prefill(int n, const float *last_row, bool with_logits);
    int score(int n, int digits, float *nll_out, int32_t *argmax_out, float *logits_out, int logits_rows, float *elapsed_ms);
    bool chain_applies(int digits) const;
    bool handover16_applies(int digits) const;
    bool hybrid_applies(size_t n_rows) const;
    int last_prefill_path() const { return last_prefill_path_; }
    int saturation_fallbacks() const { return saturation_fallbacks_; }
    int fp6_flag(int digits);
    int ensure_chain_buffers(size_t N);
    int prefill_chain_layers(size_t N);
    bool qb32_applies(int digits, size_t n_rows);
    int prefill_qb32_layers(size_t N);
    void set_phase_timing(bool on) { sp_timing_ = on; }
    void phase_times(float out[4]) const {
        for (int i = 0; i < 4; ++i) out[i] = sp_phase_us_[i];
    }
    void layer_objects(int layer, uint64_t handles[4], void *ptrs[4]) const;
    void global_objects(void *ptrs[7]) const;
    int position();
    int history(int32_t *out, int n);
    int last_logits(float *out);
    int last_hidden(float *out);
    int trace_step(const char *dir, bool with_logits);
    int probe_gateup(int reps, float *us_per_launch, double *bytes_per_launch);
    int probe_kernel(int kind, int reps, float *us_per_launch, double *bytes_per_launch);
    size_t weight_bytes() const { return weight_bytes_; }
    void *stream() const { return stream_; }

  private:
    int fail(const char *what);
    int fail_arg(const char *what);
    bool dead_ = false;
    struct Tracer;
    int step_launches(bool with_logits, int form, Tracer *tr = nullptr);
    int step_launches_reference(bool with_logits);
    int ensure_graph(bool with_logits, int form);
  public:
    int prepare_graphs(bool with_logits);
  private:
    int form_at(int pos) const;
    bool merge_ok_ = false;

    Config c_;
    std::string err_;
    void *stream_ = nullptr;
    struct Layer {
        float *attn_norm = nullptr, *ffn_norm = nullptr;
        bitnet_hip_weights_t qkv = 0, o = 0, gateup = 0, down = 0;
        float *kcache = nullptr, *vcache = nullptr;
        bool q_ok = false;
    };
    int attn_launch(Layer &L, int form, float *out, void *qout);
    int prompt_forward(int p, int n, bool with_logits, int digits, float *elapsed_ms);
    int prompt_attention(Layer &L, size_t N, void *out, bool out_f16);
    size_t pf_past_ = 0;
    void release_layer(Layer &L);
    void drop_graphs();
    int pick_token(void *stream);
    int adopt_projections(Layer &L, bitnet_hip_weights_t h[7]);
    std::vector<Layer> layers_;
    void *embed_ = nullptr;
    float *final_norm_ = nullptr;
    float *rope_sin_ = nullptr, *rope_cos_ = nullptr;
    float *x_ = nullptr, *x2_ = nullptr, *qkv_ = nullptr, *att_ = nullptr, *h_ = nullptr, *logits_ = nullptr;
    void *qa_x_ = nullptr, *qa_x2_ = nullptr, *qa_att_ = nullptr, *qa_h_ = nullptr;
    double *st_x_ = nullptr, *st_x2_ = nullptr;
    int act_mode_ = 1;
    bool kv_f16_ = false;
    std::string trace_dir_;
    float *ref_n_ = nullptr, *ref_gu_ = nullptr, *ref_t_ = nullptr;
    void *scratch_ = nullptr;
    float *attn_scratch_ = nullptr;
    int32_t *pos_ = nullptr, *n_forced_ = nullptr, *history_ = nullptr, *token_ = nullptr;
    bitnet_hip_sampler *sampler_ = nullptr;
    bool sampling_ = false;
    int host_forced_ = 0;
    int sp_cap_ = 0, sp_ctx_ = 0;
    void *sp_kv_send_ = nullptr, *sp_kv_all_ = nullptr;
    void *comm_stream_ = nullptr, *sp_ev_pack_ = nullptr, *sp_ev_gather_ = nullptr;
    int32_t *sp_block_pos_ = nullptr, *sp_tokens_ = nullptr;
    bool sp_timing_ = false;
    std::vector<void *> sp_tev_;
    float sp_phase_us_[4] = {0.f, 0.f, 0.f, 0.f};
    int pf_cap_ = 0;
    float *pf_x_ = nullptr, *pf_qkv_ = nullptr, *pf_att_ = nullptr, *pf_h_ = nullptr;
    void *pf_gemm_ws_ = nullptr, *pf_attn_ws_ = nullptr;
    int pfc_cap_ = 0;
    void *pf_xh_ = nullptr, *pf_atth_ = nullptr, *pf_hh_ = nullptr;
    float *pf_stats_ = nullptr;
    void *pf_qb_ = nullptr;
    int pf_qb_cap_ = 0;
    bool force_scaled_ = false;
    int saturation_fallbacks_ = 0;
    int sc_cap_ = 0, sc_logits_cap_ = 0;
    int32_t *sc_tgt_ = nullptr, *sc_am_ = nullptr;
    float *sc_nll_ = nullptr, *sc_logits_ = nullptr;
    void *sc_ws_ = nullptr;
    size_t sc_ws_bytes_ = 0;
    int last_prefill_path_ = 0;
    int prefill_qb32_ = -1;
    int prefill_fp6_ = -1;
    int prefill_chain_ = -1;
    size_t pf_gemm_ws_bytes_ = 0, pf_attn_ws_bytes_ = 0;
    size_t weight_bytes_ = 0;
    static constexpr int kGraphs = 6;
    void *graph_exec_[kGraphs] = {};
    void *graph_[kGraphs] = {};
    int logits_wgs_ = 512;
};

}

extern "C" {
typedef struct bitnet_host_config {
    int32_t hidden, n_layers, n_heads, n_kv_heads, head_dim, ffn, vocab, max_pos;
    float eps, rope_theta;
} bitnet_host_config;
void *bitnet_host_create(const bitnet_host_config *cfg);
void bitnet_host_destroy(void *d);
const char *bitnet_host_error(void *d);
int bitnet_host_set_layer_qk256(void *d, int layer, const float *attn_norm, const float *ffn_norm,
                                const uint8_t *q, const uint8_t *k, const uint8_t *v, const uint8_t *o,
                                const uint8_t *gate, const uint8_t *up, const uint8_t *down);
int bitnet_host_set_layer_i2s(void *d, int layer, const float *attn_norm, const float *ffn_norm,
                              const uint8_t *const *w7, const float *const *scales7, size_t block_size);
int bitnet_host_set_globals(void *d, const uint16_t *embed_f16, const float *final_norm);
int bitnet_host_reset(void *d);
int bitnet_host_set_sampling(void *d, const bitnet_hip_sampling_config *cfg);
int bitnet_host_sampling_draws(void *d, uint64_t *out);
int bitnet_host_feed(void *d, const int32_t *tokens, int n);
int bitnet_host_run(void *d, int n, int with_logits, int use_graph, float *elapsed_ms);
int bitnet_host_run_reference(void *d, int n, int with_logits);
int bitnet_host_prepare_graphs(void *d, int with_logits);
int bitnet_host_set_act_mode(void *d, int mode);
int bitnet_host_set_kv_f16(void *d, int on);
int bitnet_host_act_mode(void *d);
int bitnet_host_prefill(void *d, int n, int with_logits, int digits, float *elapsed_ms);
int bitnet_host_finish_prefill(void *d, int n, const float *last_row, int with_logits);
int bitnet_host_extend(void *d, int n, int with_logits, int digits, float *elapsed_ms);
int bitnet_host_rewind(void *d, int n);
int bitnet_host_score(void *d, int n, int digits, float *nll_out, int32_t *argmax_out, float *logits_out, int logits_rows, float *elapsed_ms);
int bitnet_host_set_phase_timing(void *d, int on);
int bitnet_host_phase_times(void *d, float out[4]);
int bitnet_host_prefill_sharded(void *d, int n, int rank, int world, bitnet_host_allgather_fn gather, void *gather_ctx, int with_logits,
                                int digits, int wire_f16, float *elapsed_ms);
int bitnet_host_rccl_allgather(void *nccl_comm, const void *send_dev, void *recv_dev, size_t bytes_per_rank, void *stream);
void bitnet_host_layer_objects(void *d, int layer, uint64_t *handles4, void **ptrs4);
void bitnet_host_global_objects(void *d, void **ptrs7);
int bitnet_host_position(void *d);
int bitnet_host_history(void *d, int32_t *out, int n);
int bitnet_host_last_logits(void *d, float *out);
int bitnet_host_last_hidden(void *d, float *out);
int bitnet_host_trace_step(void *d, const char *dir, int with_logits);
int bitnet_host_blake3_hex(const void *data, size_t len, char *out65);
int bitnet_host_probe_gateup(void *d, int reps, float *us_per_launch, double *bytes_per_launch);
int bitnet_host_probe_kernel(void *d, int kind, int reps, float *us_per_launch, double *bytes_per_launch);
uint64_t bitnet_host_weight_bytes(void *d);
}
```

### include/bitnet_hip.h

```cpp
#ifndef BITNET_HIP_H
#define BITNET_HIP_H

#include <stddef.h>
#include <stdint.h>

#ifdef __cplusplus
extern "C" {
#endif

#define BITNET_HIP_OK 0
#define BITNET_HIP_ERR_INVALID_ARGUMENT (-1)
#define BITNET_HIP_ERR_GPU (-2)
#define BITNET_HIP_ERR_UNSUPPORTED (-3)
#define BITNET_HIP_ERR_EXECUTION (-4)

#define BITNET_HIP_QTYPE_I2S 0
#define BITNET_HIP_QTYPE_TL1 1
#define BITNET_HIP_QTYPE_TL2 2


int bitnet_hip_init(int device);
void bitnet_hip_cleanup(void);
int bitnet_hip_is_available(void);
int bitnet_hip_device_count(void);
// ... 109 lines not shown
#define BITNET_HIP_FUSE_SILU_MUL 1
int bitnet_hip_gemv_fused_dev(bitnet_hip_weights_t w, const float *x_dev, float *y_dev, size_t m,
                              const float *ln_gamma_dev, float ln_eps, const float *residual_dev,
                              int flags, void *stream);
int bitnet_hip_weights_bind_ln(bitnet_hip_weights_t w, const float *ln_gamma_dev, void *stream);


int bitnet_hip_rmsnorm(const float *input, size_t in_len, const float *gamma, size_t gamma_len,
                       float *output, size_t out_len, size_t num_rows, size_t hidden_dim, float eps);
int bitnet_hip_attention(const float *q, size_t q_len, const float *k, size_t k_len, const float *v,
                         size_t v_len, float *output, size_t out_len, size_t seq_len, size_t num_heads,
                         size_t head_dim, int causal, float scale);
typedef struct bitnet_hip_gemv_item {
    const uint8_t *weights; size_t weights_len;
    const float *scales;    size_t scales_len;
    const float *input;     size_t input_len;
    float *output;          size_t output_len;
    size_t m, n, k;
} bitnet_hip_gemv_item;
int bitnet_hip_qk256_gemv_batch(const bitnet_hip_gemv_item *items, size_t n_items);
int bitnet_hip_norm_rows_dev(const float *x_dev, const float *gamma_dev, float *out_dev, size_t rows,
                             size_t hidden, float eps, int rms, void *stream);
int bitnet_hip_embed_f16_dev(const void *table_f16_dev, const int32_t *tokens_dev,
                             const int32_t *offset_dev, size_t n, size_t hidden, size_t vocab,
                             float *out_dev, void *stream);
int bitnet_hip_add_dev(const float *a_dev, const float *b_dev, float *out_dev, size_t n, void *stream);
int bitnet_hip_silu_mul_dev(const float *gate_dev, const float *up_dev, float *out_dev, size_t n, size_t tile,
                            void *stream);
int bitnet_hip_advance_pos_dev(int32_t *pos_dev, void *stream);
int bitnet_hip_attention_decode_dev(const float *qkv_dev, const float *rope_sin_dev,
                                    const float *rope_cos_dev, float *kcache_dev, float *vcache_dev,
                                    size_t n_heads, size_t n_kv_heads, size_t head_dim, size_t max_pos,
                                    const int32_t *pos_dev, float *scratch_dev, float *out_dev,
                                    void *stream);
int bitnet_hip_attention_decode_wide_dev(const float *qkv_dev, const float *rope_sin_dev,
                                         const float *rope_cos_dev, float *kcache_dev, float *vcache_dev,
                                         size_t n_heads, size_t n_kv_heads, size_t head_dim, size_t max_pos,
                                         const int32_t *pos_dev, float *scratch_dev, float *out_dev,
                                         void *stream);
int bitnet_hip_attention_decode_partial_dev(const float *qkv_dev, const float *rope_sin_dev, const float *rope_cos_dev,
                                            float *kcache_dev, float *vcache_dev, size_t n_heads, size_t n_kv_heads,
                                            size_t head_dim, size_t max_pos, const int32_t *pos_dev, float *scratch_dev,
                                            void *stream);
size_t bitnet_hip_attention_merge_max_keys(void);
int bitnet_hip_gemv_attn_merge_dev(bitnet_hip_weights_t w, const float *attn_scratch_dev, size_t n_heads,
                                   size_t n_kv_heads, size_t max_pos, const int32_t *pos_dev, float *y_dev,
                                   const float *residual_dev, void *stream);
size_t bitnet_hip_qact_bytes(size_t cols);
size_t bitnet_hip_qact_stats_bytes(size_t cols);
int bitnet_hip_quantize_act_dev(const float *x_dev, const float *gamma_dev, size_t cols, void *qact_out,
                                double *stats_out, void *stream);
int bitnet_hip_embed_q_dev(const void *table_f16_dev, const int32_t *tokens_dev, const int32_t *offset_dev,
                           size_t hidden, size_t vocab, float *x_out_dev, const float *gamma_dev, void *qact_out,
                           double *stats_out, void *stream);
int bitnet_hip_gemv_q_supported(bitnet_hip_weights_t w);
int bitnet_hip_gemv_q_dev(bitnet_hip_weights_t w, const void *qact_in, const double *stats_in,
                          const float *ln_gamma_dev, float ln_eps, const float *residual_dev, int flags,
                          float *y_dev, void *qact_out, const float *gamma_out_dev, double *stats_out, void *stream);
#define BITNET_HIP_ATTN_WIDE 1
#define BITNET_HIP_ATTN_KV_F16 2
#define BITNET_HIP_ATTN_PARTIAL 4
int bitnet_hip_attention_decode_q_dev(const float *qkv_dev, const float *rope_sin_dev, const float *rope_cos_dev,
                                      void *kcache_dev, void *vcache_dev, size_t n_heads, size_t n_kv_heads,
                                      size_t head_dim, size_t max_pos, const int32_t *pos_dev, float *scratch_dev,
                                      int flags, float *out_dev, void *qact_out, void *stream);
int bitnet_hip_attention_prefill_kv16_dev(const float *qkv_dev, const float *rope_sin_dev, const float *rope_cos_dev,
                                          void *kcache_f16_dev, void *vcache_f16_dev, size_t n_heads, size_t n_kv_heads,
                                          size_t head_dim, size_t max_pos, size_t seq_len, void *workspace_dev,
                                          size_t workspace_bytes, float *out_dev, void *stream);
#define BITNET_HIP_ATTN_CACHE_F16 1
#define BITNET_HIP_ATTN_OUT_F16 2
int bitnet_hip_attention_prefill_flags_dev(const float *qkv, const float *rope_sin, const float *rope_cos, void *kcache, void *vcache, size_t n_heads,
                                           size_t n_kv_heads, size_t head_dim, size_t max_pos, size_t seq_len, void *workspace, size_t workspace_bytes,
                                           void *out, int flags, void *stream);
size_t bitnet_hip_attention_extend_workspace_bytes(size_t n_heads, size_t n_kv_heads, size_t past_len, size_t seq_len);
int bitnet_hip_attention_extend_dev(const float *qkv_dev, const float *rope_sin_dev, const float *rope_cos_dev,
                                    void *kcache_dev, void *vcache_dev, size_t n_heads, size_t n_kv_heads, size_t head_dim,
                                    size_t max_pos, size_t past_len, size_t seq_len, void *workspace_dev, size_t workspace_bytes,
                                    void *out_dev, int flags, void *stream);
int bitnet_hip_gemv_attn_merge_q_dev(bitnet_hip_weights_t w, const float *attn_scratch_dev, size_t n_heads,
                                     size_t n_kv_heads, size_t max_pos, const int32_t *pos_dev, float *y_dev,
                                     const float *residual_dev, void *qact_out, const float *gamma_out_dev,
                                     double *stats_out, void *stream);
size_t bitnet_hip_attention_prefill_workspace_bytes(size_t n_heads, size_t n_kv_heads, size_t seq_len);
int bitnet_hip_attention_prefill_dev(const float *qkv_dev, const float *rope_sin_dev,
                                     const float *rope_cos_dev, float *kcache_dev, float *vcache_dev,
                                     size_t n_heads, size_t n_kv_heads, size_t head_dim, size_t max_pos,
                                     size_t seq_len, void *workspace_dev, size_t workspace_bytes,
                                     float *out_dev, void *stream);
size_t bitnet_hip_attention_prefill_sharded_workspace_bytes(size_t n_heads, size_t n_kv_heads, size_t n_q, size_t n_ctx);
int bitnet_hip_attention_prefill_sharded_dev(const float *q_dev, size_t ld_q, const int32_t *q_block_pos_dev,
                                             size_t n_q, const float *kv_dev, size_t ld_kv, size_t n_ctx,
                                             const float *rope_sin_dev, const float *rope_cos_dev,
                                             float *kcache_dev, float *vcache_dev, size_t n_heads,
                                             size_t n_kv_heads, size_t head_dim, size_t max_pos,
                                             void *workspace_dev, size_t workspace_bytes, float *out_dev,
                                             void *stream);
int bitnet_hip_attention_prefill_gathered_dev(const float *q_dev, size_t ld_q, const int32_t *q_block_pos_dev, size_t n_q,
                                              const void *kv_gathered_dev, size_t n_ctx, size_t world, int kv_is_f16,
                                              const float *rope_sin_dev, const float *rope_cos_dev, void *kcache_dev,
                                              void *vcache_dev, int cache_f16, size_t n_heads, size_t n_kv_heads,
                                              size_t head_dim, size_t max_pos, void *workspace_dev, size_t workspace_bytes,
                                              float *out_dev, void *stream);
int bitnet_hip_attention_prefill_gathered_phase_dev(const float *q_dev, size_t ld_q, const int32_t *q_block_pos_dev, size_t n_q,
                                                    const void *kv_gathered_dev, size_t n_ctx, size_t world, int kv_is_f16,
                                                    const float *rope_sin_dev, const float *rope_cos_dev, void *kcache_dev,
                                                    void *vcache_dev, int cache_f16, size_t n_heads, size_t n_kv_heads,
                                                    size_t head_dim, size_t max_pos, void *workspace_dev, size_t workspace_bytes,
                                                    float *out_dev, int phase, void *stream);
int bitnet_hip_pack_cols_dev(const float *src_dev, size_t ld, size_t col0, size_t ncols, size_t rows, void *dst_dev,
                             int as_f16, void *stream);
size_t bitnet_hip_attention_scratch_bytes(size_t n_kv_heads, size_t max_pos);
int bitnet_hip_logits_f16_dev(const void *table_f16_dev, const float *x_dev, const float *gamma_dev,
                              float eps, size_t hidden, size_t vocab, float *logits_dev,
                              void *scratch_dev, size_t n_workgroups, int32_t *token_dev,
                              int32_t *pos_dev, int32_t *history_dev, const int32_t *n_forced_dev,
                              void *stream);
int bitnet_hip_argmax_dev(const float *v_dev, size_t n, void *scratch_dev, size_t n_workgroups,
                          int32_t *token_dev, void *stream);

size_t bitnet_hip_score_workspace_bytes(size_t n_rows, size_t hidden, size_t vocab);
int bitnet_hip_score_f16_dev(const void *table_f16_dev, const float *x_dev, const float *gamma_dev, float eps, size_t hidden, size_t vocab,
                             size_t n_rows, const int32_t *targets_dev, float *nll_dev, int32_t *argmax_dev, float *logits_dev,
                             size_t logits_rows, void *workspace_dev, size_t workspace_bytes, void *stream);

#define BITNET_HIP_SAMPLE_SMALL_K 64
typedef struct bitnet_hip_sampling_config {
    float temperature;
    int32_t top_k;
    float top_p;
    float repetition_penalty;
    uint64_t seed;
} bitnet_hip_sampling_config;
typedef struct bitnet_hip_sampler bitnet_hip_sampler;
int bitnet_hip_sampler_create(size_t vocab, const bitnet_hip_sampling_config *cfg, bitnet_hip_sampler **out);
void bitnet_hip_sampler_destroy(bitnet_hip_sampler *sampler);
int bitnet_hip_sampler_configure(bitnet_hip_sampler *sampler, const bitnet_hip_sampling_config *cfg);
int bitnet_hip_sampler_reset(bitnet_hip_sampler *sampler);
int bitnet_hip_sampler_draws(bitnet_hip_sampler *sampler, uint64_t *draws);
int bitnet_hip_sample_dev(bitnet_hip_sampler *sampler, const float *logits_dev, size_t vocab, int32_t *token_dev,
                          int32_t *pos_dev, int32_t *history_dev, const int32_t *n_forced_dev, void *stream);
int bitnet_hip_sample_host(bitnet_hip_sampler *sampler, const float *logits, size_t vocab, const uint32_t *generated,
                           size_t n_generated, uint32_t *token);

int bitnet_hip_hbm_read_ceiling(size_t bytes, int iters, double *best_gbs, double *mean_gbs, void *stream);

#ifdef __cplusplus
}
#endif
#endif
```

Measured before the change: 1209 tokens/s.

## Extend fused attention-merge o_proj GEMV to eight chunk records up to 512 keys

Adds a third decode form that keeps the partial-attention path, with its merge fused into the quantised o_proj GEMV, for contexts up to 512 keys by combining up to eight 64-key chunk records instead of four. The merge prologue now loads per-head max and sum through scalar (uniform) loads, handles a tail element group for 2560-column matrices, and computes the exp weights once per lane and broadcasts them with readlane. It is meant to avoid the separate wide or unfused attention path and its extra output write and quantise launch for keys between 257 and 512. In exchange it adds more register pressure from the eight-record arrays, two extra graph slots, and an exact-exp path when more than four chunks are combined.

```diff
diff --git a/bitnet-rs_amd/__init__.py b/bitnet-rs_amd/__init__.py
--- a/bitnet-rs_amd/__init__.py
+++ b/bitnet-rs_amd/__init__.py
@@ -124,6 +124,9 @@
         L.bitnet_hip_gemv_q_dev.argtypes = [C.c_uint64, _vp, _vp, _vp, C.c_float, _vp, C.c_int, _vp, _vp, _vp, _vp, _vp]
         L.bitnet_hip_attention_decode_q_dev.argtypes = [_vp, _vp, _vp, _vp, _vp, _sz, _sz, _sz, _sz, _vp, _vp, C.c_int, _vp, _vp, _vp]
         L.bitnet_hip_gemv_attn_merge_q_dev.argtypes = [C.c_uint64, _vp, _sz, _sz, _sz, _vp, _vp, _vp, _vp, _vp, _vp, _vp]
+        L.bitnet_hip_gemv_attn_merge_rec_q_dev.argtypes = [C.c_uint64, _vp, _sz, _sz, _sz, _vp, _vp, _vp, _vp, _vp, _vp, _sz, _vp]
+        L.bitnet_hip_attention_merge_q_max_keys.restype = _sz
+        L.bitnet_hip_attention_merge_q_max_keys.argtypes = []
         L.bitnet_hip_matmul_workspace_bytes.argtypes = [_sz, _sz, C.c_int]
         L.bitnet_hip_matmul_workspace_bytes.restype = _sz
         L.bitnet_hip_matmul_fused_dev.argtypes = [C.c_uint64, _vp, _vp, _sz, _vp, C.c_float, _vp, C.c_int, C.c_int, _vp, _sz, _vp]
@@ -475,6 +478,14 @@
         self._check(self.c.bitnet_hip_attention_decode_q_dev(_ptr(qkv), _ptr(rope_sin), _ptr(rope_cos), _ptr(kcache), _ptr(vcache), n_heads, n_kv,
                                                              head_dim, max_pos, _ptr(pos), _ptr(scratch), flags, _optr(out), _optr(qact_out), _vp(stream)))
 
+    def attention_merge_q_max_keys(self) -> int:
+        return int(self.c.bitnet_hip_attention_merge_q_max_keys())
+
+    def gemv_attn_merge_rec_q_dev(self, h: int, scratch, n_heads, n_kv, max_pos, pos, y, qact_out, max_records: int, residual=None, gamma_out=None,
+                                  stats_out=None, stream: int = 0) -> None:
+        self._check(self.c.bitnet_hip_gemv_attn_merge_rec_q_dev(h, _ptr(scratch), n_heads, n_kv, max_pos, _ptr(pos), _ptr(y), _optr(residual),
+                                                                _ptr(qact_out), _optr(gamma_out), _optr(stats_out), max_records, _vp(stream)))
+
     def gemv_attn_merge_q_dev(self, h: int, scratch, n_heads, n_kv, max_pos, pos, y, qact_out, residual=None, gamma_out=None, stats_out=None,
                               stream: int = 0) -> None:
         self._check(self.c.bitnet_hip_gemv_attn_merge_q_dev(h, _ptr(scratch), n_heads, n_kv, max_pos, _ptr(pos), _ptr(y), _optr(residual),
@@ -753,6 +764,7 @@
         L.bitnet_host_set_act_mode.argtypes = [C.c_void_p, C.c_int]
         L.bitnet_host_act_mode.argtypes = [C.c_void_p]
         L.bitnet_host_position.argtypes = [C.c_void_p]
+        L.bitnet_host_form_at.argtypes = [C.c_void_p, C.c_int]
         L.bitnet_host_last_prefill_path.argtypes = [C.c_void_p]
         L.bitnet_host_saturation_fallbacks.argtypes = [C.c_void_p]
         L.bitnet_host_history.argtypes = [C.c_void_p, C.POINTER(C.c_int32), C.c_int]
@@ -930,6 +942,9 @@
     def position(self) -> int:
         return int(self.c.bitnet_host_position(self.h))
 
+    def form_at(self, pos: int) -> int:
+        return int(self.c.bitnet_host_form_at(self.h, pos))
+
     def history(self, n: int) -> np.ndarray:
         out = np.zeros(n, np.int32)
         self._check(self.c.bitnet_host_history(self.h, out.ctypes.data_as(C.POINTER(C.c_int32)), n))
diff --git a/bitnet-rs_amd/csrc/abi.hip b/bitnet-rs_amd/csrc/abi.hip
--- a/bitnet-rs_amd/csrc/abi.hip
+++ b/bitnet-rs_amd/csrc/abi.hip
@@ -940,10 +940,11 @@
 }
 
 size_t bitnet_hip_attention_merge_max_keys(void) { return (size_t)4 * 64; }
+size_t bitnet_hip_attention_merge_q_max_keys(void) { return (size_t)8 * 64; }
 
 static int gemv_attn_merge(bitnet_hip_weights_t h, const float *attn_scratch_dev, size_t n_heads, size_t n_kv_heads, size_t max_pos,
                            const int32_t *pos_dev, float *y_dev, const float *residual_dev, void *qact_out, const float *gamma_out_dev,
-                           double *stats_out, void *stream, int chunk_log2 = 6) {
+                           double *stats_out, void *stream, int chunk_log2 = 6, int records = 4) {
     BH_GUARD_BEGIN
     const WeightsRef w = lookup(h);
     if (!w) return set_error(BITNET_HIP_ERR_INVALID_ARGUMENT, "unknown weights handle %llu", (unsigned long long)h);
@@ -956,6 +957,9 @@
         return set_error(BITNET_HIP_ERR_UNSUPPORTED, "gemv_attn_merge_dev: matrix shape %zux%zu not supported", w->rows, w->cols);
     if (qact_out && w->rows % 16 != 0)
         return set_error(BITNET_HIP_ERR_UNSUPPORTED, "gemv_attn_merge_q_dev: rows %zu must be a multiple of 16 for a QAct output", w->rows);
+    if (records != 4 && !(qact_out && gemvq_supported(*w) && w->cols <= 2560))
+        return set_error(BITNET_HIP_ERR_UNSUPPORTED, "gemv_attn_merge_rec_q_dev: %d records need a QAct matrix of at most 2560 columns (got %zux%zu)", records,
+                         w->rows, w->cols);
     if (qact_out && gemvq_supported(*w) && w->cols <= 4096) {
         GemvQIo io;
         io.residual = residual_dev;
@@ -968,6 +972,7 @@
         io.attn_chunk_log2 = chunk_log2;
         io.attn_chunks_max = (int)div_ceil(max_pos, (size_t)1 << chunk_log2);
         io.attn_group_log2 = group == 4 ? 2 : group == 2 ? 1 : 0;
+        io.attn_records = records;
         hipError_t e = launch_gemv_q(*w, io, (hipStream_t)stream);
         if (e != hipSuccess) return set_error(BITNET_HIP_ERR_GPU, "kernel launch failed: %s", hipGetErrorString(e));
         return BITNET_HIP_OK;
@@ -996,6 +1001,16 @@
                                      const float *gamma_out_dev, double *stats_out, void *stream) {
     if (!qact_out) return set_error(BITNET_HIP_ERR_INVALID_ARGUMENT, "Null pointer passed to gemv_attn_merge_q_dev");
     return gemv_attn_merge(h, attn_scratch_dev, n_heads, n_kv_heads, max_pos, pos_dev, y_dev, residual_dev, qact_out, gamma_out_dev, stats_out, stream);
+}
+
+int bitnet_hip_gemv_attn_merge_rec_q_dev(bitnet_hip_weights_t h, const float *attn_scratch_dev, size_t n_heads, size_t n_kv_heads,
+                                         size_t max_pos, const int32_t *pos_dev, float *y_dev, const float *residual_dev, void *qact_out,
+                                         const float *gamma_out_dev, double *stats_out, size_t max_records, void *stream) {
+    if (!qact_out) return set_error(BITNET_HIP_ERR_INVALID_ARGUMENT, "Null pointer passed to gemv_attn_merge_rec_q_dev");
+    if (max_records != 4 && max_records != 8)
+        return set_error(BITNET_HIP_ERR_INVALID_ARGUMENT, "gemv_attn_merge_rec_q_dev: max_records must be 4 or 8 (got %zu)", max_records);
+    return gemv_attn_merge(h, attn_scratch_dev, n_heads, n_kv_heads, max_pos, pos_dev, y_dev, residual_dev, qact_out, gamma_out_dev, stats_out, stream, 6,
+                           (int)max_records);
 }
 
 
diff --git a/bitnet-rs_amd/csrc/common.hpp b/bitnet-rs_amd/csrc/common.hpp
--- a/bitnet-rs_amd/csrc/common.hpp
+++ b/bitnet-rs_amd/csrc/common.hpp
@@ -108,6 +108,7 @@
     const float *attn_rec = nullptr;
     const int *attn_pos = nullptr;
     int attn_chunks_max = 0, attn_group_log2 = 0, attn_chunk_log2 = 6;
+    int attn_records = 4;
 };
 
 
diff --git a/bitnet-rs_amd/csrc/kernels_gemvq.hip b/bitnet-rs_amd/csrc/kernels_gemvq.hip
--- a/bitnet-rs_amd/csrc/kernels_gemvq.hip
+++ b/bitnet-rs_amd/csrc/kernels_gemvq.hip
@@ -20,6 +20,13 @@
     do {             \
     } while (0)
 #endif
+
+__device__ __forceinline__ v2f load_uniform2(const void *p) {
+    return *reinterpret_cast<const __attribute__((address_space(4))) v2f *>(reinterpret_cast<uintptr_t>(p));
+}
+__device__ __forceinline__ int load_uniform_i(const int *p) {
+    return *reinterpret_cast<const __attribute__((address_space(4))) int *>(reinterpret_cast<uintptr_t>(p));
+}
 
 struct GemvQArgs {
     const uint8_t *tiles;
@@ -45,7 +52,7 @@
     unsigned long long *stamps;
 };
 
-template <int NW, int RING, int SC, int LN, int NCP, int NE = 0>
+template <int NW, int RING, int SC, int LN, int NCP, int NE = 0, int NE1 = 0, int NR = 4>
 __global__ __launch_bounds__(NW * 64) void k_gemv_q(GemvQArgs p) {
     constexpr int NT = NW * 64;
     constexpr bool MRG = NE > 0;
@@ -73,24 +80,57 @@
 
     const uint32_t q_last = (uint32_t)kQRec * (uint32_t)p.nblk - 16u;
     v4u qa[NCP];
-    float4 mo[MRG ? NE : 1][4];
-    float2 mml[MRG ? NE : 1][4];
+    float4 mo[MRG ? NE : 1][NR];
+    float mt[NE1 ? NE1 : 1][NR];
+    v2f sml[MRG ? NE : 1][2][NR];
+    v2f smt[NE1 ? NE1 : 1][NR];
+    int mpos = 0;
     if (!MRG) {
 #pragma unroll
         for (int i = 0; i < NCP; ++i) qa[i] = *reinterpret_cast<const v4u *>(p.qin + umin32(16u * (uint32_t)(tid + NT * i), q_last));
     } else {
+        const int gl = p.attn_group_log2, gm = (1 << gl) - 1, h_last = (p.cols >> 7) - 1;
+        const uint32_t kv_stride = (uint32_t)p.attn_chunks_max * (kAttnRecFloats * 4u);
+        const char *rbase = reinterpret_cast<const char *>(p.attn_rec);
+        uint32_t ro[NR];
+#pragma unroll
+        for (int c = 0; c < NR; ++c) ro[c] = (uint32_t)(c < p.attn_chunks_max ? c : p.attn_chunks_max - 1) * (kAttnRecFloats * 4u);
+        mpos = load_uniform_i(p.attn_pos);
 #pragma unroll
         for (int i = 0; i < NE; ++i) {
             int e = 4 * (tid + NT * i);
             e = e < p.cols ? e : p.cols - 4;
-            const int h = e >> 7, d = e & 127, kvh = h >> p.attn_group_log2, hg = h & ((1 << p.attn_group_log2) - 1);
-            const float *rb = p.attn_rec + (size_t)kvh * p.attn_chunks_max * kAttnRecFloats;
-#pragma unroll
-            for (int c = 0; c < 4; ++c) {
-                const float *rec = rb + (size_t)(c < p.attn_chunks_max ? c : p.attn_chunks_max - 1) * kAttnRecFloats;
-                mml[i][c] = *reinterpret_cast<const float2 *>(rec + 2 * hg);
-                mo[i][c] = *reinterpret_cast<const float4 *>(rec + 2 * kMaxGroupQ + hg * 128 + d);
-            }
+            const int h = e >> 7, d = e & 127;
+            const uint32_t vo = (uint32_t)(h >> gl) * kv_stride + 4u * (uint32_t)(2 * kMaxGroupQ + (h & gm) * 128 + d);
+#pragma unroll
+            for (int c = 0; c < NR; ++c) mo[i][c] = *reinterpret_cast<const float4 *>(rbase + (vo + ro[c]));
+        }
+#pragma unroll
+        for (int i = 0; i < NE1; ++i) {
+            int e = 4 * NT * NE + tid + NT * i;
+            e = e < p.cols ? e : p.cols - 1;
+            const int h = e >> 7, d = e & 127;
+            const uint32_t vo = (uint32_t)(h >> gl) * kv_stride + 4u * (uint32_t)(2 * kMaxGroupQ + (h & gm) * 128 + d);
+#pragma unroll
+            for (int c = 0; c < NR; ++c) mt[i][c] = *reinterpret_cast<const float *>(rbase + (vo + ro[c]));
+        }
+#pragma unroll
+        for (int i = 0; i < NE; ++i)
+#pragma unroll
+            for (int s = 0; s < 2; ++s) {
+                int hs = 2 * (wave + NW * i) + s;
+                hs = hs < h_last ? hs : h_last;
+                const uint32_t so = (uint32_t)(hs >> gl) * kv_stride + 8u * (uint32_t)(hs & gm);
+#pragma unroll
+                for (int c = 0; c < NR; ++c) sml[i][s][c] = load_uniform2(rbase + (so + ro[c]));
+            }
+#pragma unroll
+        for (int i = 0; i < NE1; ++i) {
+            int hs = ((4 * NT * NE + NT * i) >> 7) + (wave >> 1);
+            hs = hs < h_last ? hs : h_last;
+            const uint32_t so = (uint32_t)(hs >> gl) * kv_stride + 8u * (uint32_t)(hs & gm);
+#pragma unroll
+            for (int c = 0; c < NR; ++c) smt[i][c] = load_uniform2(rbase + (so + ro[c]));
         }
     }
     v4u st = {0u, 0u, 0u, 0u};
@@ -139,26 +179,57 @@
 #pragma unroll
         for (int i = 0; i < NCP; ++i) *reinterpret_cast<v4u *>(cq + 16 * (tid + NT * i)) = qa[i];
     } else {
-        const int m_chunks = (*p.attn_pos + (1 << p.attn_chunk_log2)) >> p.attn_chunk_log2;
+        const int m_chunks = (mpos + (1 << p.attn_chunk_log2)) >> p.attn_chunk_log2;
+        const bool as_combine = NR > 4 && m_chunks > 4;
+        constexpr int NS = MRG ? NE + NE1 : 1;
+        float ml[NS][NR], xl[NS][NR], wl[NS][NR];
+#pragma unroll
+        for (int k = 0; k < NS; ++k) {
+            float mc[NR], M = -INFINITY;
+#pragma unroll
+            for (int c = 0; c < NR; ++c) {
+                const float mv = k < NE ? (lane < 32 ? sml[k < NE ? k : 0][0][c].x : sml[k < NE ? k : 0][1][c].x) : smt[k < NE ? 0 : k - NE][c].x;
+                ml[k][c] = k < NE ? (lane < 32 ? sml[k < NE ? k : 0][0][c].y : sml[k < NE ? k : 0][1][c].y) : smt[k < NE ? 0 : k - NE][c].y;
+                mc[c] = c < m_chunks ? mv : -INFINITY;
+                M = fmaxf(M, mc[c]);
+            }
+#pragma unroll
+            for (int c = 0; c < NR; ++c) xl[k][c] = mc[c] - M;
+        }
+        if constexpr (NR <= 4) {
+#pragma unroll
+            for (int k = 0; k < NS; ++k)
+#pragma unroll
+                for (int c = 0; c < NR; ++c) wl[k][c] = __expf(xl[k][c]);
+        } else {
+            float tx = 0.0f;
+#pragma unroll
+            for (int k = 0; k < NS; ++k)
+#pragma unroll
+                for (int c = 0; c < NR; ++c) tx = (lane & 31) == 8 * k + c ? xl[k][c] : tx;
+            const float ex = as_combine ? expf(tx) : __expf(tx);
+#pragma unroll
+            for (int k = 0; k < NS; ++k)
+#pragma unroll
+                for (int c = 0; c < NR; ++c) {
+                    const float lo = readlane_f(ex, 8 * k + c);
+                    wl[k][c] = k < NE ? (lane < 32 ? lo : readlane_f(ex, 32 + 8 * k + c)) : lo;
+                }
+        }
 #pragma unroll
         for (int i = 0; i < NE; ++i) {
             const int e = 4 * (tid + NT * i);
-            float M = -INFINITY;
-#pragma unroll
-            for (int c = 0; c < 4; ++c) {
-                mml[i][c].x = c < m_chunks ? mml[i][c].x : -INFINITY;
-                M = fmaxf(M, mml[i][c].x);
-            }
             float L = 0.0f;
             float4 a = {0.0f, 0.0f, 0.0f, 0.0f};
 #pragma unroll
-            for (int c = 0; c < 4; ++c) {
-                const float w = __expf(mml[i][c].x - M);
-                L += w * mml[i][c].y;
-                a.x += w * mo[i][c].x, a.y += w * mo[i][c].y, a.z += w * mo[i][c].z, a.w += w * mo[i][c].w;
+            for (int c = 0; c < NR; ++c) {
+                const float w = wl[i][c];
+                L = fmaf(w, ml[i][c], L);
+                a.x = fmaf(w, mo[i][c].x, a.x), a.y = fmaf(w, mo[i][c].y, a.y), a.z = fmaf(w, mo[i][c].z, a.z), a.w = fmaf(w, mo[i][c].w, a.w);
             }
             const float rl = e < p.cols ? 1.0f / L : 0.0f;
-            const float v[4] = {a.x * rl, a.y * rl, a.z * rl, a.w * rl};
+            float v[4] = {a.x * rl, a.y * rl, a.z * rl, a.w * rl};
+            if (as_combine && e < p.cols) v[0] = a.x / L, v[1] = a.y / L, v[2] = a.z / L, v[3] = a.w / L;
             uint32_t u = __float_as_uint(fmaxf(fmaxf(fabsf(v[0]), fabsf(v[1])), fmaxf(fabsf(v[2]), fabsf(v[3])))), o;
             o = dpp_u<0xB1>(u), u = o > u ? o : u;
             o = dpp_u<0x4E>(u), u = o > u ? o : u;
@@ -179,6 +250,31 @@
                 *reinterpret_cast<uint32_t *>(qb + 16 * tp + (e & 15)) = d0;
                 *reinterpret_cast<uint32_t *>(qb + 256 + 16 * tp + (e & 15)) = d1;
                 if ((e & 15) == 0) reinterpret_cast<float *>(qb + 512)[4 * (tp >> 2) + 2 * (tp & 1) + ((tp & 3) >> 1)] = as;
+            }
+        }
+#pragma unroll
+        for (int i = 0; i < NE1; ++i) {
+            const int e = 4 * NT * NE + tid + NT * i;
+            float L = 0.0f, a = 0.0f;
+#pragma unroll
+            for (int c = 0; c < NR; ++c) {
+                const float w = wl[NE + i][c];
+                L = fmaf(w, ml[NE + i][c], L);
+                a = fmaf(w, mt[i][c], a);
+            }
+            float v = a * (e < p.cols ? 1.0f / L : 0.0f);
+            if (as_combine && e < p.cols) v = a / L;
+            int be = (int)(__float_as_uint(row16_max_abs(v)) >> 23);
+            be = be < 32 ? 32 : be;
+            be = be > 254 ? 254 : be;
+            const float sc = __uint_as_float((uint32_t)(267 - be) << 23), as = __uint_as_float((uint32_t)(be - 13) << 23);
+            const uint32_t t = ((uint32_t)qcvt_rpi(v * sc) + 0x80u) ^ 0x80u;
+            if (e < p.cols) {
+                const int grp = e >> 4, rec = grp >> 4, tp = grp & 15, r = e & 15;
+                uint8_t *qb = cq + kQRec * rec;
+                qb[16 * tp + r] = (uint8_t)t;
+                qb[256 + 16 * tp + r] = (uint8_t)(t >> 8);
+                if (r == 0) reinterpret_cast<float *>(qb + 512)[4 * (tp >> 2) + 2 * (tp & 1) + ((tp & 3) >> 1)] = as;
             }
         }
     }
@@ -393,12 +489,17 @@
 #undef BH_QPICK
 #undef BH_QPICK2
     if (io.attn_rec) {
-        const int ne = (int)div_ceil(w.cols / 4, (size_t)512);
-        if (ln || nw != 8 || ring > 2 || ncp != 1 || w.cols % 128 != 0 || ne > 2 || !io.attn_pos || io.attn_chunks_max < 1) return hipErrorInvalidValue;
-#define BH_QMRG(NEv)                                                                                                                   \
-    if (ne <= NEv && !kfn) kfn = sc == 2 ? k_gemv_q<8, 2, 2, 0, 1, NEv> : sc == 1 ? k_gemv_q<8, 2, 1, 0, 1, NEv> : k_gemv_q<8, 2, 0, 0, 1, NEv>;
+        const int nr = io.attn_records;
+        const int ne = w.cols <= 2560 ? 1 : 2, ne1 = w.cols > 2048 && w.cols <= 2560 ? 1 : 0;
+        if (ln || nw != 8 || ring > 2 || ncp != 1 || w.cols % 128 != 0 || w.cols > 4096 || !io.attn_pos || io.attn_chunks_max < 1 || (nr != 4 && nr != 8) ||
+            (nr == 8 && ne == 2))
+            return hipErrorInvalidValue;
+        if (((uint64_t)(w.cols / 128) >> io.attn_group_log2) * (uint64_t)io.attn_chunks_max * kAttnRecFloats * 4u >= (1ull << 32)) return hipErrorInvalidValue;
+#define BH_QMRG(NEv, NE1v, NRv)                     \
+    if (ne == NEv && ne1 == NE1v && nr == NRv)      \
+        kfn = sc == 2 ? k_gemv_q<8, 2, 2, 0, 1, NEv, NE1v, NRv> : sc == 1 ? k_gemv_q<8, 2, 1, 0, 1, NEv, NE1v, NRv> : k_gemv_q<8, 2, 0, 0, 1, NEv, NE1v, NRv>;
         kfn = nullptr;
-        BH_QMRG(1) BH_QMRG(2)
+        BH_QMRG(1, 0, 4) BH_QMRG(1, 1, 4) BH_QMRG(2, 0, 4) BH_QMRG(1, 0, 8) BH_QMRG(1, 1, 8)
 #undef BH_QMRG
     }
     if (!kfn) return hipErrorInvalidValue;
diff --git a/bitnet-rs_amd/host/decoder.cpp b/bitnet-rs_amd/host/decoder.cpp
--- a/bitnet-rs_amd/host/decoder.cpp
+++ b/bitnet-rs_amd/host/decoder.cpp
@@ -99,6 +99,7 @@
         const int group = c_.n_kv_heads > 0 ? c_.n_heads / c_.n_kv_heads : 0;
         merge_ok_ = c_.head_dim == 128 && (group == 1 || group == 2 || group == 4) && c_.n_heads % c_.n_kv_heads == 0 &&
                     (size_t)c_.n_heads * 128 <= 4096;
+        merge8_ok_ = merge_ok_ && (size_t)c_.n_heads * 128 <= 2560;
     }
     bool ok = true;
     ok &= dalloc(&x_, H) == hipSuccess && dalloc(&x2_, H) == hipSuccess;
@@ -405,7 +406,7 @@
 }
 
 int Decoder::attn_launch(Layer &L, int form, float *out, void *qout) {
-    const int flags = (form >= 2 ? BITNET_HIP_ATTN_WIDE : 0) | ((form & 1) ? BITNET_HIP_ATTN_PARTIAL : 0) | (kv_f16_ ? BITNET_HIP_ATTN_KV_F16 : 0);
+    const int flags = (form == 2 ? BITNET_HIP_ATTN_WIDE : 0) | ((form & 1) ? BITNET_HIP_ATTN_PARTIAL : 0) | (kv_f16_ ? BITNET_HIP_ATTN_KV_F16 : 0);
     BCHK(bitnet_hip_attention_decode_q_dev(qkv_, rope_sin_, rope_cos_, L.kcache, L.vcache, (size_t)c_.n_heads, (size_t)c_.n_kv_heads, (size_t)c_.head_dim,
                                            (size_t)c_.max_pos, pos_, attn_scratch_, flags, out, qout, stream_));
     return 0;
@@ -470,7 +471,8 @@
     const size_t H = c_.hidden;
     const size_t tQD = (size_t)c_.n_heads * c_.head_dim, tKD = (size_t)c_.n_kv_heads * c_.head_dim;
     const std::string tp = tr ? "t" + std::to_string(tr->seq) + "/" : "";
-    if (tr && (form & 1)) form -= 1;
+    if (tr && (form & 1)) form = 0;
+    if (form == 3 && !qact_path()) form = 0;
     if (qact_path()) {
         const size_t NH = (size_t)c_.n_heads, NK = (size_t)c_.n_kv_heads, MP = (size_t)c_.max_pos;
         BCHK(bitnet_hip_embed_q_dev(embed_, history_, pos_, H, (size_t)c_.vocab, x_, layers_[0].attn_norm, qa_x_, st_x_, s));
@@ -482,9 +484,9 @@
             TRACE(bp + "q_proj", "q_proj", (int)l, qkv_, tQD);
             TRACE(bp + "k_proj", "k_proj", (int)l, qkv_ + tQD, tKD);
             TRACE(bp + "v_proj", "v_proj", (int)l, qkv_ + tQD + tKD, tKD);
-            if (form == 1) {
-                if (int rc = attn_launch(L, 1, nullptr, nullptr)) return rc;
-                BCHK(bitnet_hip_gemv_attn_merge_q_dev(L.o, attn_scratch_, NH, NK, MP, pos_, x2_, x_, qa_x2_, L.ffn_norm, st_x2_, s));
+            if (form & 1) {
+                if (int rc = attn_launch(L, form, nullptr, nullptr)) return rc;
+                BCHK(bitnet_hip_gemv_attn_merge_rec_q_dev(L.o, attn_scratch_, NH, NK, MP, pos_, x2_, x_, qa_x2_, L.ffn_norm, st_x2_, form == 3 ? 8 : 4, s));
             } else {
                 if (int rc = attn_launch(L, form, tr ? att_ : nullptr, qa_att_)) return rc;
                 TRACE(bp + "attn_out", "attn_out", (int)l, att_, tQD);
@@ -625,10 +627,11 @@
 }
 
 int Decoder::form_at(int pos) const {
-    static const bool merge_env = !(getenv("BITNET_HOST_ATTN_MERGE") && atoi(getenv("BITNET_HOST_ATTN_MERGE")) == 0);
+    static const int merge_env = getenv("BITNET_HOST_ATTN_MERGE") ? atoi(getenv("BITNET_HOST_ATTN_MERGE")) : 8;
     static const bool wide_env = !(getenv("BITNET_HOST_ATTN_WIDE") && atoi(getenv("BITNET_HOST_ATTN_WIDE")) == 0);
     const int keys = pos + 1;
-    if (merge_env && merge_ok_ && keys <= (int)bitnet_hip_attention_merge_max_keys()) return 1;
+    if (merge_env > 0 && merge_ok_ && keys <= (int)bitnet_hip_attention_merge_max_keys()) return 1;
+    if (merge_env >= 8 && merge8_ok_ && qact_path() && keys <= kMerge8MaxKeys && keys <= (int)bitnet_hip_attention_merge_q_max_keys()) return 3;
     if (wide_env && c_.n_kv_heads * ((keys + 63) / 64) > 256) return 2;
     return 0;
 }
@@ -1598,6 +1601,7 @@
     if (Decoder *D = live(d)) D->global_objects(ptrs7);
 }
 int bitnet_host_position(void *d) { LIVE(-1); return D->position(); }
+int bitnet_host_form_at(void *d, int pos) { LIVE(-1); return pos < 0 ? -1 : D->form_at(pos); }
 int bitnet_host_last_prefill_path(void *d) { LIVE(-1); return D->last_prefill_path(); }
 int bitnet_host_saturation_fallbacks(void *d) { LIVE(-1); return D->saturation_fallbacks(); }
 int bitnet_host_history(void *d, int32_t *out, int n) { LIVE(BITNET_HIP_ERR_INVALID_ARGUMENT); return D->history(out, n); }
diff --git a/bitnet-rs_amd/host/decoder.hpp b/bitnet-rs_amd/host/decoder.hpp
--- a/bitnet-rs_amd/host/decoder.hpp
+++ b/bitnet-rs_amd/host/decoder.hpp
@@ -110,9 +110,11 @@
     int ensure_graph(bool with_logits, int form);
   public:
     int prepare_graphs(bool with_logits);
+    int form_at(int pos) const;
+    static constexpr int kMerge8MaxKeys = 512;
   private:
-    int form_at(int pos) const;
     bool merge_ok_ = false;
+    bool merge8_ok_ = false;
 
     Config c_;
     std::string err_;
@@ -176,7 +178,7 @@
     int prefill_chain_ = -1;
     size_t pf_gemm_ws_bytes_ = 0, pf_attn_ws_bytes_ = 0;
     size_t weight_bytes_ = 0;
-    static constexpr int kGraphs = 6;
+    static constexpr int kGraphs = 8;
     void *graph_exec_[kGraphs] = {};
     void *graph_[kGraphs] = {};
     int logits_wgs_ = 512;
@@ -221,6 +223,7 @@
 void bitnet_host_layer_objects(void *d, int layer, uint64_t *handles4, void **ptrs4);
 void bitnet_host_global_objects(void *d, void **ptrs7);
 int bitnet_host_position(void *d);
+int bitnet_host_form_at(void *d, int pos);
 int bitnet_host_history(void *d, int32_t *out, int n);
 int bitnet_host_last_logits(void *d, float *out);
 int bitnet_host_last_hidden(void *d, float *out);
diff --git a/include/bitnet_hip.h b/include/bitnet_hip.h
--- a/include/bitnet_hip.h
+++ b/include/bitnet_hip.h
@@ -215,6 +215,11 @@
                                      size_t n_kv_heads, size_t max_pos, const int32_t *pos_dev, float *y_dev,
                                      const float *residual_dev, void *qact_out, const float *gamma_out_dev,
                                      double *stats_out, void *stream);
+size_t bitnet_hip_attention_merge_q_max_keys(void);
+int bitnet_hip_gemv_attn_merge_rec_q_dev(bitnet_hip_weights_t w, const float *attn_scratch_dev, size_t n_heads,
+                                         size_t n_kv_heads, size_t max_pos, const int32_t *pos_dev, float *y_dev,
+                                         const float *residual_dev, void *qact_out, const float *gamma_out_dev,
+                                         double *stats_out, size_t max_records, void *stream);
 size_t bitnet_hip_attention_prefill_workspace_bytes(size_t n_heads, size_t n_kv_heads, size_t seq_len);
 int bitnet_hip_attention_prefill_dev(const float *qkv_dev, const float *rope_sin_dev,
                                      const float *rope_cos_dev, float *kcache_dev, float *vcache_dev,
```

After: 1229 tokens/s, median of 6. 1.6% higher.
